# qiutang98/chord

Hardware: AMD Instinct MI355X
Metric: Gtri/s into 4K 64-bit visbuffer (higher is better)
Workload: dtype f32+u64; 1 GPU; street_4k_hzb; scene_triangles_lod0=2799616, objects=352, hzb=True, cull=flat, parallelism=single

## Files before the change

### chord_amd/csrc/kernels_raster.hip

```cpp

#include "device_layer.h"
#include "device_math.h"

#include <algorithm>
#include <cstdlib>
#include <cstring>
#include <type_traits>

namespace chord {

#define GUARD_BAND 1024.0f
#define LDS_VERTS 256
#define TILE CHORD_TILE
#define TILE_SHIFT CHORD_TILE_SHIFT
#define TPITCH (TILE + 1)
#define SMALL_AREA 256
#define TC_STRIDE CHORD_TILECOUNT_STRIDE
#define TC_BLOCKS 1u
#define TC_TICKET 2u
#ifndef CHORD_MASKED_FUSED
#define CHORD_MASKED_FUSED 1
#endif
#define TC_MASKED 3u

struct RasterParams {
    const uint32_t* count; const ChordDrawCmd* cmds;
    uint32_t cmdCap;
    uint32_t* leftCount; ChordDrawCmd* leftCmds;
    const DObjFrame* objFrame; const DObjStatic* objStatic;
    const DMeshlet* meshlets; const uint32_t* meshletData; const float* positions;
    const DMaterial* materials; const uint8_t* texAlpha; const float* texcoords;
    unsigned long long* vis;
    float* depthOut;
    float W, H; int32_t Wi, Hi;
    ShardInfo shard;
    TriRec* tris; uint32_t triCap;
    TriRecC* trisC; uint32_t triCapC;
    uint32_t* tileCount; uint32_t* tileBins; uint32_t binCap; uint32_t tilesX, tilesY;
    uint32_t* binPool; uint32_t binPoolChunks; uint32_t* binPoolCount;
    unsigned long long* binChunkTab; uint32_t binStamp; uint32_t binMaxChunks;
    unsigned long long* blockPool; uint32_t blockCap;
    uint32_t blockForce;
    ClipTri* clipTris; uint32_t clipTriCap; uint32_t pass;
    uint32_t* largeList; uint32_t largeCap;
    DeviceCounters* counters;
    uint2* tileOrder;
    unsigned long long* tileSlabs;
    uint32_t hzbFused;
    ChordHZBDesc hzbDesc;
    uint16_t* hzbMinA;
    uint16_t* hzbMinB; uint16_t* hzbMaxB;
    uint16_t* hzbExA;
    uint16_t* hzbExB;
    uint32_t* tileRange;
    unsigned long long* tileClocks;
    unsigned long long* tilePhase;
    uint32_t depthOnly, depthClamp;
    float biasConst, biasSlope;
    uint32_t clearTiles;
    uint32_t* binHint;
    uint32_t* countHint;
    uint32_t slotHot;
    uint32_t* hotTiles;
    uint32_t tileSlots;
    uint32_t tileSplitMin, tileSliceLen;
    uint2* tileOrderNext;
    uint32_t orderAll;
    uint32_t orderKept;
    uint32_t* heavyHint;
    uint32_t* tileTouched;
    uint32_t debug;
};
#define ABL(p, flag) (RASTER_ABLATION && ((p).debug & (flag)) != 0u)
#define DBG_NO_PIXELS   1u
#define DBG_NO_BIN      2u
#define DBG_TILE_CLOCKS 16u
#define DBG_NO_OUT      128u
#define DBG_NO_HZB      256u
#define DBG_SETUP_CLOCKS 512u
#define DBG_NO_VIS_STORE 1024u
#define DBG_NO_SPLIT    2048u
#define DBG_NO_TINY     32u
#define DBG_TILE_EXIT   64u
#define DBG_NO_ENTRY    8192u
#define DBG_NO_BATCH    16384u
#define DBG_NO_UNITS    4096u
#define DBG_SKIP_LIGHT  1048576u
#define DBG_SKIP_HEAVY  2097152u

template <typename T>
__device__ __forceinline__ T scalar_load(const T* ptr)
{
    return *reinterpret_cast<const __attribute__((address_space(4))) T*>(reinterpret_cast<uintptr_t>(ptr));
}
__device__ __forceinline__ const RasterParams* kernel_args()
{
    unsigned long long kp = (unsigned long long)__builtin_amdgcn_kernarg_segment_ptr();
    asm volatile("" : "+s"(kp));
    return reinterpret_cast<const RasterParams*>(kp);
}

__device__ __forceinline__ uint32_t mbcnt64(unsigned long long m) { return __builtin_amdgcn_mbcnt_hi((uint32_t)(m >> 32), __builtin_amdgcn_mbcnt_lo((uint32_t)m, 0u)); }
__device__ __forceinline__ int32_t bcast(int32_t v, int src) { return __builtin_amdgcn_readlane(v, src); }
__device__ __forceinline__ uint32_t bcast(uint32_t v, int src) { return (uint32_t)__builtin_amdgcn_readlane((int)v, src); }
__device__ __forceinline__ float bcast(float v, int src) { return __int_as_float(__builtin_amdgcn_readlane(__float_as_int(v), src)); }

__device__ __forceinline__ bool owns_tile(const ShardInfo& s, int32_t tx, int32_t ty)
{
    if (s.ranks <= 1) return true;
    return shard_owns_tile(s, (uint32_t)tx, (uint32_t)ty);
}
__device__ __forceinline__ bool owns_rect(const ShardInfo& s, int32_t px0, int32_t py0, int32_t px1, int32_t py1)
{
    if (s.ranks <= 1) return true;
    return shard_owns_any_tile(s, (uint32_t)px0 >> TILE_SHIFT, (uint32_t)py0 >> TILE_SHIFT, (uint32_t)px1 >> TILE_SHIFT, (uint32_t)py1 >> TILE_SHIFT);
}

__device__ __forceinline__ bool in_fast_volume_xy(const f4& h)
{
    return h.w > 0.0f && (GUARD_BAND * h.w + h.x) >= 0.0f && (GUARD_BAND * h.w - h.x) >= 0.0f &&
           (GUARD_BAND * h.w + h.y) >= 0.0f && (GUARD_BAND * h.w - h.y) >= 0.0f;
}

__device__ __forceinline__ bool in_fast_volume(const f4& h)
{
    return h.w > 0.0f && (h.w - h.z) >= 0.0f && h.z >= 0.0f &&
           (GUARD_BAND * h.w + h.x) >= 0.0f && (GUARD_BAND * h.w - h.x) >= 0.0f &&
           (GUARD_BAND * h.w + h.y) >= 0.0f && (GUARD_BAND * h.w - h.y) >= 0.0f;
}

struct TriSetup {
    int32_t X[3], Y[3];
    float d0, e1, e2, invA;
    int32_t px0, py0, px1, py1;
    int64_t area;
    int32_t s;
    uint32_t payload;
};

__device__ __forceinline__ bool narrow_extent(const TriSetup& ts)
{
    const int32_t extX = max(ts.X[0], max(ts.X[1], ts.X[2])) - min(ts.X[0], min(ts.X[1], ts.X[2]));
    const int32_t extY = max(ts.Y[0], max(ts.Y[1], ts.Y[2])) - min(ts.Y[0], min(ts.Y[1], ts.Y[2]));
    return extX <= (1 << 14) && extY <= (1 << 14);
}

__device__ __forceinline__ bool fits_compact(const TriSetup& ts)
{
    return narrow_extent(ts);
}

__device__ __forceinline__ void write_record_c(TriRecC* dst, const TriSetup& ts, const float d[3])
{
    TriRecC r;
    r.X0 = ts.X[0]; r.Y0 = ts.Y[0];
    r.dX1 = (int16_t)(ts.X[1] - ts.X[0]); r.dY1 = (int16_t)(ts.Y[1] - ts.Y[0]);
    r.dX2 = (int16_t)(ts.X[2] - ts.X[0]); r.dY2 = (int16_t)(ts.Y[2] - ts.Y[0]);
    r.d[0] = d[0]; r.d[1] = d[1]; r.d[2] = d[2];
    r.payload = ts.payload;
    *dst = r;
}

__device__ __forceinline__ bool tri_setup(TriSetup& ts, bool twoSided, int32_t Wi, int32_t Hi)
{
    const int32_t dx1 = ts.X[1] - ts.X[0], dy1 = ts.Y[1] - ts.Y[0], dx2 = ts.X[2] - ts.X[0], dy2 = ts.Y[2] - ts.Y[0];
    int64_t area2;
    const bool small = (uint32_t)(dx1 + 32767) < 65535u && (uint32_t)(dy1 + 32767) < 65535u &&
                       (uint32_t)(dx2 + 32767) < 65535u && (uint32_t)(dy2 + 32767) < 65535u;
    const bool allSmall = __ballot(!small) == 0ull;
    if (allSmall) area2 = (int64_t)(__mul24(dx1, dy2) - __mul24(dx2, dy1));
    else area2 = (int64_t)dx1 * (int64_t)dy2 - (int64_t)dx2 * (int64_t)dy1;
    if (area2 == 0) return false;
    if (!twoSided && area2 > 0) return false;
    ts.s = area2 < 0 ? -1 : 1;
    ts.area = area2 < 0 ? -area2 : area2;
    const int32_t minX = min(ts.X[0], min(ts.X[1], ts.X[2])), maxX = max(ts.X[0], max(ts.X[1], ts.X[2]));
    const int32_t minY = min(ts.Y[0], min(ts.Y[1], ts.Y[2])), maxY = max(ts.Y[0], max(ts.Y[1], ts.Y[2]));
    ts.px0 = max(0, (minX + 127) >> 8);
    ts.py0 = max(0, (minY + 127) >> 8);
    ts.px1 = min(Wi - 1, (maxX - 128) >> 8);
    ts.py1 = min(Hi - 1, (maxY - 128) >> 8);
    if (ts.px1 < ts.px0 || ts.py1 < ts.py0) return false;
    if (allSmall) ts.invA = 1.0f / (float)(int32_t)ts.area;
    else ts.invA = 1.0f / (float)(double)ts.area;
    return true;
}

__device__ __forceinline__ float depth_bias(const TriSetup& ts, const float d[3], float biasConst, float biasSlope)
{
    const int64_t s = ts.s;
    const float invA = ts.invA;
    const int64_t a1 = -s * (int64_t)(ts.Y[0] - ts.Y[2]), b1 = s * (int64_t)(ts.X[0] - ts.X[2]);
    const int64_t a2 = -s * (int64_t)(ts.Y[1] - ts.Y[0]), b2 = s * (int64_t)(ts.X[1] - ts.X[0]);
    const float e1 = d[1] - d[0], e2 = d[2] - d[0];
    const float dzdx = ((float)(double)(a1 * 256) * invA) * e1 + ((float)(double)(a2 * 256) * invA) * e2;
    const float dzdy = ((float)(double)(b1 * 256) * invA) * e1 + ((float)(double)(b2 * 256) * invA) * e2;
    const float m = fmaxf(fabsf(dzdx), fabsf(dzdy));
    const float mz = fmaxf(fabsf(d[0]), fmaxf(fabsf(d[1]), fabsf(d[2])));
    const int32_t e = (int32_t)((__float_as_uint(mz) >> 23) & 0xFFu) - 23;
    const float r = (e > 0 && e < 255) ? __uint_as_float((uint32_t)e << 23) : 0.0f;
    return biasSlope * m + biasConst * r;
}

__device__ __forceinline__ void tri_setup_from_compact(TriSetup& ts, const TriRecC& r, int32_t Wi, int32_t Hi)
{
    ts.X[0] = r.X0; ts.Y[0] = r.Y0;
    ts.X[1] = r.X0 + r.dX1; ts.Y[1] = r.Y0 + r.dY1;
    ts.X[2] = r.X0 + r.dX2; ts.Y[2] = r.Y0 + r.dY2;
    ts.payload = r.payload;
    const int32_t area2 = (int32_t)r.dX1 * (int32_t)r.dY2 - (int32_t)r.dX2 * (int32_t)r.dY1;
    ts.s = area2 < 0 ? -1 : 1;
    ts.invA = 1.0f / (float)(area2 < 0 ? -area2 : area2);
    ts.d0 = r.d[0]; ts.e1 = r.d[1] - r.d[0]; ts.e2 = r.d[2] - r.d[0];
    const int32_t minX = min(ts.X[0], min(ts.X[1], ts.X[2])), maxX = max(ts.X[0], max(ts.X[1], ts.X[2]));
    const int32_t minY = min(ts.Y[0], min(ts.Y[1], ts.Y[2])), maxY = max(ts.Y[0], max(ts.Y[1], ts.Y[2]));
    ts.px0 = max(0, (minX + 127) >> 8);
    ts.py0 = max(0, (minY + 127) >> 8);
    ts.px1 = min(Wi - 1, (maxX - 128) >> 8);
    ts.py1 = min(Hi - 1, (maxY - 128) >> 8);
    ts.area = 0;
}

__device__ __forceinline__ void tri_setup_from_record(TriSetup& ts, const TriRec& r, int32_t Wi, int32_t Hi)
{
#pragma unroll
    for (int i = 0; i < 3; i++) { ts.X[i] = r.X[i]; ts.Y[i] = r.Y[i]; }
    ts.payload = r.payload;
    ts.s = (r.twoSided & 2u) ? -1 : 1;
    ts.invA = __uint_as_float(r.pad);
    ts.d0 = r.d[0]; ts.e1 = r.d[1] - r.d[0]; ts.e2 = r.d[2] - r.d[0];
    const int32_t minX = min(ts.X[0], min(ts.X[1], ts.X[2])), maxX = max(ts.X[0], max(ts.X[1], ts.X[2]));
    const int32_t minY = min(ts.Y[0], min(ts.Y[1], ts.Y[2])), maxY = max(ts.Y[0], max(ts.Y[1], ts.Y[2]));
    ts.px0 = max(0, (minX + 127) >> 8);
    ts.py0 = max(0, (minY + 127) >> 8);
    ts.px1 = min(Wi - 1, (maxX - 128) >> 8);
    ts.py1 = min(Hi - 1, (maxY - 128) >> 8);
    ts.area = 0;
}



struct RecordEmitParams {
    DeviceCounters* counters; ClipTri* clipTris; uint32_t clipTriCap; uint32_t pass;
    TriRec* tris; uint32_t triCap; TriRecC* trisC; uint32_t triCapC; uint32_t* largeList; uint32_t largeCap;
    uint32_t* tileCount; uint32_t* tileBins; uint32_t binCap; uint32_t tilesX;
    uint32_t* binPool; uint32_t binPoolChunks; uint32_t* binPoolCount;
    unsigned long long* binChunkTab; uint32_t binStamp; uint32_t binMaxChunks;
    uint32_t* tileTouched;
    ShardInfo shard;
};
__device__ __forceinline__ RecordEmitParams load_record_emit_params()
{
    const RasterParams* q = kernel_args();
    RecordEmitParams e;
    e.counters = scalar_load(&q->counters); e.clipTris = scalar_load(&q->clipTris); e.clipTriCap = scalar_load(&q->clipTriCap); e.pass = scalar_load(&q->pass);
    e.tris = scalar_load(&q->tris); e.triCap = scalar_load(&q->triCap); e.trisC = scalar_load(&q->trisC); e.triCapC = scalar_load(&q->triCapC);
    e.largeList = scalar_load(&q->largeList); e.largeCap = scalar_load(&q->largeCap);
    e.tileCount = scalar_load(&q->tileCount); e.tileBins = scalar_load(&q->tileBins); e.binCap = scalar_load(&q->binCap); e.tilesX = scalar_load(&q->tilesX);
    e.binPool = scalar_load(&q->binPool); e.binPoolChunks = scalar_load(&q->binPoolChunks); e.binPoolCount = scalar_load(&q->binPoolCount);
    e.binChunkTab = scalar_load(&q->binChunkTab); e.binStamp = scalar_load(&q->binStamp); e.binMaxChunks = scalar_load(&q->binMaxChunks);
    e.tileTouched = scalar_load(&q->tileTouched);
    e.shard.ranks = scalar_load(&q->shard.ranks); e.shard.rank = scalar_load(&q->shard.rank); e.shard.slotsPerRank = 0u; e.shard.tilesX = 0u;
    e.shard.ownedRows = scalar_load(&q->shard.ownedRows); e.shard.tileSlot = nullptr;
    return e;
}

struct BinElect { int leader; uint32_t rank, group; };

__device__ __forceinline__ BinElect wave_bin_elect(bool has, uint32_t tile, uint32_t lane)
{
    BinElect e; e.leader = 0; e.rank = 0; e.group = 0;
    unsigned long long todo = __ballot(has);
    const unsigned long long lt = (1ull << lane) - 1ull;
    while (todo) {
        const int l = __ffsll((long long)todo) - 1;
        const uint32_t k = bcast(tile, l);
        const unsigned long long same = __ballot(has && tile == k);
        if (has && tile == k) { e.leader = l; e.rank = (uint32_t)__popcll(same & lt); e.group = (uint32_t)__popcll(same); }
        todo &= ~same;
    }
    return e;
}

__device__ __forceinline__ uint32_t bin_capacity(const RasterParams& p) { return p.binCap + p.binMaxChunks * CHORD_BIN_CHUNK; }

template <class P>
__device__ __forceinline__ void bin_alloc(const P& p, uint32_t tile, uint32_t slot)
{
    if (slot == 0u && p.tileTouched) atomicOr(&p.tileTouched[tile >> 5], 1u << (tile & 31u));
#ifdef EXP_NO_CHUNKS
    return;
#endif
    if (slot < p.binCap) return;
    const uint32_t o = slot - p.binCap, j = o >> CHORD_BIN_CHUNK_SHIFT;
    if (j >= p.binMaxChunks || (o & (CHORD_BIN_CHUNK - 1u)) != 0u) return;
    uint32_t id = atomicAdd(p.binPoolCount, 1u);
    if (id >= p.binPoolChunks) { id = CHORD_BIN_CHUNK_INVALID; atomicOr(&p.counters->overflow, 1u); }
    __hip_atomic_store(p.binChunkTab + (__umul24(tile, p.binMaxChunks) + j), ((unsigned long long)p.binStamp << 32) | id,
                       __ATOMIC_RELAXED, __HIP_MEMORY_SCOPE_AGENT);
}

template <class P>
__device__ __forceinline__ void bin_put(const P& p, uint32_t tile, uint32_t slot, uint32_t gi)
{
#ifdef EXP_NO_CHUNKS
    slot &= p.binCap - 1u;
#endif
    if (slot < p.binCap) { p.tileBins[__umul24(tile, p.binCap) + slot] = gi; return; }
    const uint32_t o = slot - p.binCap, j = o >> CHORD_BIN_CHUNK_SHIFT;
    if (j >= p.binMaxChunks) { atomicOr(&p.counters->overflow, 1u); return; }
    const unsigned long long* ent = p.binChunkTab + (__umul24(tile, p.binMaxChunks) + j);
    const unsigned long long stamp = (unsigned long long)p.binStamp << 32;
    unsigned long long e = 0;
    uint32_t spins = 0;
    for (;;) {
        e = __hip_atomic_load(ent, __ATOMIC_RELAXED, __HIP_MEMORY_SCOPE_AGENT);
        if ((e & 0xFFFFFFFF00000000ull) == stamp) break;
        if (++spins > (1u << 20)) { atomicOr(&p.counters->overflow, 4u); return; }
        __builtin_amdgcn_s_sleep(4);
    }
    const uint32_t id = (uint32_t)e;
    if (id != CHORD_BIN_CHUNK_INVALID) p.binPool[((size_t)id << CHORD_BIN_CHUNK_SHIFT) + (o & (CHORD_BIN_CHUNK - 1u))] = gi;
}

__device__ __forceinline__ void bin_store(const RasterParams& p, uint32_t tile, uint32_t slot, uint32_t gi)
{
    bin_alloc(p, tile, slot);
    bin_put(p, tile, slot, gi);
}

struct BinTicket {
    uint32_t tileA[4], tileB[4], slotA[4], slotB[4];
    uint32_t has;
    uint32_t eA[4], eB[4];
};

template <class P>
__device__ __forceinline__ void wave_bin_issue(const P& p, bool emitA, const TriSetup& tsA, bool emitB, const TriSetup& tsB,
                                               uint32_t lane, BinTicket& k, const bool masked = false)
{
    auto tile_of = [&](const TriSetup& ts, int r, bool emit, uint32_t& tile) -> bool {
        const int32_t tx0 = ts.px0 >> TILE_SHIFT, tx1 = ts.px1 >> TILE_SHIFT, ty0 = ts.py0 >> TILE_SHIFT, ty1 = ts.py1 >> TILE_SHIFT;
        const int32_t tx = (r & 1) ? tx1 : tx0, ty = (r & 2) ? ty1 : ty0;
        bool has = emit && !((r & 1) && tx1 == tx0) && !((r & 2) && ty1 == ty0);
        if (has) has = owns_tile(p.shard, tx, ty);
        tile = has ? __umul24((uint32_t)ty, p.tilesX) + (uint32_t)tx : 0u;
        return has;
    };
    k.has = 0u;
#pragma unroll
    for (int r = 0; r < 4; r++) {
        k.slotA[r] = 0u; k.slotB[r] = 0u;
        if (tile_of(tsA, r, emitA, k.tileA[r])) k.has |= 1u << r;
        if (tile_of(tsB, r, emitB, k.tileB[r])) k.has |= 16u << r;
    }
#pragma unroll
    for (int r = 0; r < 4; r++) {
        const BinElect a = wave_bin_elect((k.has & (1u << r)) != 0u, k.tileA[r], lane);
        const BinElect b = wave_bin_elect((k.has & (16u << r)) != 0u, k.tileB[r], lane);
        k.eA[r] = (uint32_t)a.leader | a.rank << 8; k.eB[r] = (uint32_t)b.leader | b.rank << 8;
        if ((k.has & (1u << r)) && (int)lane == a.leader) k.slotA[r] = atomicAdd(&p.tileCount[(size_t)k.tileA[r] * TC_STRIDE], a.group);
        if ((k.has & (16u << r)) && (int)lane == b.leader) k.slotB[r] = atomicAdd(&p.tileCount[(size_t)k.tileB[r] * TC_STRIDE], b.group);
    }
    if (masked) {
#pragma unroll
        for (int r = 0; r < 4; r++) {
            if ((k.has & (1u << r)) && lane == (k.eA[r] & 0xFFu)) p.tileCount[(size_t)k.tileA[r] * TC_STRIDE + TC_MASKED] = 1u;
            if ((k.has & (16u << r)) && lane == (k.eB[r] & 0xFFu)) p.tileCount[(size_t)k.tileB[r] * TC_STRIDE + TC_MASKED] = 1u;
        }
    }
}

template <class P>
__device__ __forceinline__ void wave_bin_commit(const P& p, BinTicket& k, bool okA, uint32_t giA, bool okB, uint32_t giB)
{
#pragma unroll
    for (int r = 0; r < 4; r++) {
        k.slotA[r] = __shfl(k.slotA[r], (int)(k.eA[r] & 0xFFu), 64) + (k.eA[r] >> 8);
        k.slotB[r] = __shfl(k.slotB[r], (int)(k.eB[r] & 0xFFu), 64) + (k.eB[r] >> 8);
    }
    if (k.has) {
#pragma unroll
        for (int r = 0; r < 4; r++) {
            if (k.has & (1u << r)) bin_alloc(p, k.tileA[r], k.slotA[r]);
            if (k.has & (16u << r)) bin_alloc(p, k.tileB[r], k.slotB[r]);
        }
    }
#pragma unroll
    for (int r = 0; r < 4; r++) {
        if (okA && (k.has & (1u << r))) bin_put(p, k.tileA[r], k.slotA[r], giA);
        if (okB && (k.has & (16u << r))) bin_put(p, k.tileB[r], k.slotB[r], giB);
    }
}

__device__ __forceinline__ bool touches_many_tiles(const TriSetup& ts)
{
    return ((ts.px1 >> TILE_SHIFT) - (ts.px0 >> TILE_SHIFT)) > 1 || ((ts.py1 >> TILE_SHIFT) - (ts.py0 >> TILE_SHIFT)) > 1;
}

__device__ __forceinline__ void write_record(TriRec* dst, const TriSetup& ts, const float d[3], bool twoSided, bool masked = false)
{
    TriRec r;
#pragma unroll
    for (int i = 0; i < 3; i++) { r.X[i] = ts.X[i]; r.Y[i] = ts.Y[i]; r.d[i] = d[i]; }
    r.payload = ts.payload;
    r.twoSided = (twoSided ? 1u : 0u) | (ts.s < 0 ? 2u : 0u) | (masked ? 4u : 0u);
    r.pad = __float_as_uint(ts.invA);
    *dst = r;
}

__device__ __forceinline__ bool filter_is_linear(uint32_t f)
{
    return f == CHORD_FILTER_LINEAR || f == CHORD_FILTER_LINEAR_MIPMAP_NEAREST || f == CHORD_FILTER_LINEAR_MIPMAP_LINEAR;
}

__device__ __forceinline__ uint32_t mask_level_filter(const DMaterial& m, int64_t absArea2, const float u[3], const float v[3])
{
    uint32_t level = 0u;
    bool linear = filter_is_linear(m.magFilter);
    if (m.texOffset != 0xFFFFFFFFu) {
        const float texels = (float)m.texWidth * (float)m.texHeight;
        const float auv = fabsf((u[1] - u[0]) * (v[2] - v[0]) - (u[2] - u[0]) * (v[1] - v[0])) * texels;
        const float apx = (float)(double)absArea2 * (1.0f / 65536.0f);
        const float ratio = auv / apx;
        if (ratio >= 1.0f) {
            const int32_t e = (int32_t)((__float_as_uint(ratio) >> 23) & 0xFFu) - 127;
            level = min((uint32_t)(e >> 1), m.texMips - 1u);
            linear = filter_is_linear(m.minFilter);
        }
    }
    return level | (linear ? 256u : 0u);
}

__device__ __forceinline__ void write_mask_ext(TriRec* slot, const DMaterial* mp, uint32_t material, int64_t absArea2,
                                               const float u[3], const float v[3], const float w[3])
{
    DMaterial m;
    m.texOffset = mp->texOffset; m.texWidth = mp->texWidth; m.texHeight = mp->texHeight; m.texMips = mp->texMips;
    m.minFilter = mp->minFilter; m.magFilter = mp->magFilter; m.wrapS = mp->wrapS; m.wrapT = mp->wrapT;
    m.alphaFactor = mp->alphaFactor; m.alphaCutOff = mp->alphaCutOff;
    TriRecMaskExt e;
#pragma unroll
    for (int i = 0; i < 3; i++) { e.iw[i] = 1.0f / w[i]; e.uw[i] = u[i] * e.iw[i]; e.vw[i] = v[i] * e.iw[i]; }
    e.levelFilter = mask_level_filter(m, absArea2, u, v);
    (void)material;
    const uint32_t level = e.levelFilter & 0xFFu;
    e.levelBase = 0xFFFFFFFFu; e.dims = 0u; e.magicS = e.biasS = e.magicT = e.biasT = 0u;
    if (m.texOffset != 0xFFFFFFFFu) {
        const DMatLevel L = mp->levels[level];
        e.levelBase = L.base; e.dims = L.dims;
        e.magicS = L.magicS; e.biasS = L.biasS; e.magicT = L.magicT; e.biasT = L.biasT;
    }
    e.wraps = (m.wrapS & 0xFFFFu) | m.wrapT << 16;
    e.alphaFactor = m.alphaFactor; e.alphaCutOff = m.alphaCutOff;
    uint4* dst = reinterpret_cast<uint4*>(slot);
    const uint4* src = reinterpret_cast<const uint4*>(&e);
    dst[0] = src[0]; dst[1] = src[1]; dst[2] = src[2]; dst[3] = src[3];
    reinterpret_cast<uint32_t*>(slot)[16] = e.biasS; reinterpret_cast<uint32_t*>(slot)[17] = e.magicT; reinterpret_cast<uint32_t*>(slot)[18] = e.biasT;
}

#ifndef EXP_MASKED
#define EXP_MASKED 0
#endif
__device__ __forceinline__ int32_t period_mod(int32_t i, int32_t period, uint32_t magic, uint32_t bias)
{
    if ((EXP_MASKED & 4) || magic == 0u) return i & (period - 1);
    const uint32_t iu = (uint32_t)i + bias;
    uint32_t r = iu - __umulhi(iu, magic) * (uint32_t)period;
    if (r >= (uint32_t)period) r -= (uint32_t)period;
    return (int32_t)r;
}
__device__ __forceinline__ int32_t wrap_index(int32_t i, int32_t n, uint32_t mode, uint32_t magic, uint32_t bias)
{
    if (mode == CHORD_WRAP_CLAMP_TO_EDGE) return i < 0 ? 0 : (i > n - 1 ? n - 1 : i);
    if (mode == CHORD_WRAP_MIRRORED_REPEAT) {
        const int32_t m = period_mod(i, 2 * n, magic, bias);
        return m < n ? m : 2 * n - 1 - m;
    }
    return period_mod(i, n, magic, bias);
}

__device__ __forceinline__ void wrap_pair(int32_t i, int32_t n, uint32_t mode, uint32_t magic, uint32_t bias, int32_t& w0, int32_t& w1)
{
    if (mode == CHORD_WRAP_CLAMP_TO_EDGE) {
        w0 = i < 0 ? 0 : (i > n - 1 ? n - 1 : i);
        w1 = i + 1 < 0 ? 0 : (i + 1 > n - 1 ? n - 1 : i + 1);
        return;
    }
    const bool mirror = mode == CHORD_WRAP_MIRRORED_REPEAT;
    const int32_t period = mirror ? 2 * n : n;
    const int32_t m = period_mod(i, period, magic, bias);
    const int32_t m1 = m + 1 == period ? 0 : m + 1;
    w0 = mirror ? (m < n ? m : 2 * n - 1 - m) : m;
    w1 = mirror ? (m1 < n ? m1 : 2 * n - 1 - m1) : m1;
}

__device__ __forceinline__ int32_t texel_floor(float x)
{
    if (!(fabsf(x) < 1.0e9f)) return 0;
    return (int32_t)floorf(x);
}

struct AlphaLevel {
    const uint8_t* base;
    int32_t W, H;
    float fW, fH;
    uint32_t wrapS, wrapT;
    uint32_t magicS, biasS, magicT, biasT;
    bool linear;
};
__device__ __forceinline__ AlphaLevel alpha_level(const uint8_t* __restrict__ texAlpha, const TriRecMaskExt& e)
{
    const uint32_t levelBase = e.levelBase, dims = e.dims;
    AlphaLevel a;
    a.base = nullptr; a.W = 1; a.H = 1; a.fW = 1.0f; a.fH = 1.0f; a.wrapS = e.wraps & 0xFFFFu; a.wrapT = e.wraps >> 16; a.linear = (e.levelFilter & 256u) != 0u;
    a.magicS = e.magicS; a.biasS = e.biasS; a.magicT = e.magicT; a.biasT = e.biasT;
    if (levelBase == 0xFFFFFFFFu) return a;
    a.W = (int32_t)(dims & 0xFFFFu) + 1; a.H = (int32_t)(dims >> 16) + 1;
    a.fW = (float)a.W; a.fH = (float)a.H;
    a.base = texAlpha + levelBase;
    return a;
}
__device__ __forceinline__ float sample_alpha(const AlphaLevel& t, float u, float v)
{
    if (!t.base) return 1.0f;
    if (EXP_MASKED & 1) return 1.0f;
    if (!t.linear || (EXP_MASKED & 2)) {
        const int32_t ix = wrap_index(texel_floor(u * t.fW), t.W, t.wrapS, t.magicS, t.biasS), iy = wrap_index(texel_floor(v * t.fH), t.H, t.wrapT, t.magicT, t.biasT);
        return (float)t.base[iy * t.W + ix] * (1.0f / 255.0f);
    }
    const float x = u * t.fW - 0.5f, y = v * t.fH - 0.5f;
    const int32_t x0 = texel_floor(x), y0 = texel_floor(y);
    float fx = x - (float)x0, fy = y - (float)y0;
    if (!(fabsf(x) < 1.0e9f)) fx = 0.0f;
    if (!(fabsf(y) < 1.0e9f)) fy = 0.0f;
    int32_t ix0, ix1, iy0, iy1;
    wrap_pair(x0, t.W, t.wrapS, t.magicS, t.biasS, ix0, ix1);
    wrap_pair(y0, t.H, t.wrapT, t.magicT, t.biasT, iy0, iy1);
    const float a00 = (float)t.base[iy0 * t.W + ix0] * (1.0f / 255.0f), a10 = (float)t.base[iy0 * t.W + ix1] * (1.0f / 255.0f);
    const float a01 = (float)t.base[iy1 * t.W + ix0] * (1.0f / 255.0f), a11 = (float)t.base[iy1 * t.W + ix1] * (1.0f / 255.0f);
    const float top = a00 + (a10 - a00) * fx, bot = a01 + (a11 - a01) * fx;
    return top + (bot - top) * fy;
}

__device__ __forceinline__ void setup_emit_mask_ext(const RasterParams& p, TriRec* slot, uint32_t triWord, const float uv[6],
                                                 const float* lW, uint32_t material, int64_t absArea2)
{
    float u[3], v[3], w[3];
#pragma unroll
    for (int i = 0; i < 3; i++) {
        u[i] = uv[2 * i]; v[i] = uv[2 * i + 1];
        w[i] = lW[(triWord >> (8 * i)) & 0xFFu];
    }
    write_mask_ext(slot, &p.materials[material], material, absArea2, u, v, w);
}

template <int PITCH>
__device__ __forceinline__ void tile_raster_narrow(unsigned long long* tile, const TriSetup& ts, int32_t ox, int32_t oy,
                                                   int32_t x0, int32_t y0, int32_t x1, int32_t y1, bool noPixels, const bool clampZ);

__device__ __forceinline__ void wave_min2_max2(int32_t& a, int32_t& b, int32_t& c, int32_t& d)
{
#define DPP_STEP(ctrl)                                                \
    "v_min_i32_dpp %0, %0, %0 " ctrl "\n\t"                           \
    "v_min_i32_dpp %1, %1, %1 " ctrl "\n\t"                           \
    "v_max_i32_dpp %2, %2, %2 " ctrl "\n\t"                           \
    "v_max_i32_dpp %3, %3, %3 " ctrl "\n\t"
    asm volatile("s_nop 1\n\t"
                 DPP_STEP("quad_perm:[1,0,3,2] row_mask:0xf bank_mask:0xf")
                 DPP_STEP("quad_perm:[2,3,0,1] row_mask:0xf bank_mask:0xf")
                 DPP_STEP("row_ror:4 row_mask:0xf bank_mask:0xf")
                 DPP_STEP("row_ror:8 row_mask:0xf bank_mask:0xf")
                 DPP_STEP("row_bcast:15 row_mask:0xa bank_mask:0xf")
                 DPP_STEP("row_bcast:31 row_mask:0xc bank_mask:0xf")
                 "s_nop 0"
                 : "+v"(a), "+v"(b), "+v"(c), "+v"(d));
#undef DPP_STEP
    a = __builtin_amdgcn_readlane(a, 63); b = __builtin_amdgcn_readlane(b, 63);
    c = __builtin_amdgcn_readlane(c, 63); d = __builtin_amdgcn_readlane(d, 63);
}

__device__ __forceinline__ void wave_sum2(uint32_t& a, uint32_t& b)
{
#define DPP_STEP(ctrl)                                                \
    "v_add_u32_dpp %0, %0, %0 " ctrl "\n\t"                           \
    "v_add_u32_dpp %1, %1, %1 " ctrl "\n\t"
    asm volatile("s_nop 1\n\t"
                 DPP_STEP("quad_perm:[1,0,3,2] row_mask:0xf bank_mask:0xf") "s_nop 0\n\t"
                 DPP_STEP("quad_perm:[2,3,0,1] row_mask:0xf bank_mask:0xf") "s_nop 0\n\t"
                 DPP_STEP("row_ror:4 row_mask:0xf bank_mask:0xf") "s_nop 0\n\t"
                 DPP_STEP("row_ror:8 row_mask:0xf bank_mask:0xf") "s_nop 0\n\t"
                 DPP_STEP("row_bcast:15 row_mask:0xa bank_mask:0xf") "s_nop 0\n\t"
                 DPP_STEP("row_bcast:31 row_mask:0xc bank_mask:0xf")
                 "s_nop 0"
                 : "+v"(a), "+v"(b));
#undef DPP_STEP
    a = (uint32_t)__builtin_amdgcn_readlane((int)a, 63); b = (uint32_t)__builtin_amdgcn_readlane((int)b, 63);
}

enum { K_NONE = 0, K_EMIT = 1, K_CLIP = 2 };
#define WIN CHORD_BLOCK_WIN
#define DBG_NO_BLOCKS 32768u
#define DBG_FORCE_BLOCKS 65536u
#define DBG_FORCE_HOT 262144u

template <bool MASKED>
__device__ __forceinline__ void raster_setup_body(const RasterParams& p, const ChordDrawCmd* __restrict__ cmds, const uint32_t count, float (*sVert)[4][LDS_VERTS],
                                                  const uint32_t firstCmd0, const uint32_t firstCmd1, const uint32_t firstCmd2, const bool firstCmdValid)
{
    const uint32_t lane = threadIdx.x & 63u, wave = threadIdx.x >> 6;
    float* lX = sVert[0][wave]; float* lY = sVert[1][wave]; float* lW = sVert[2][wave];
    float* lU = sVert[3][wave]; float* lV = sVert[4][wave]; float* lD = sVert[5][wave];

    const uint32_t listShard = (blockIdx.x * 4u + wave) % CHORD_LIST_SHARDS;

    struct Header {
        uint32_t objectId, meshletId, slot, V, T, dataOffset, vertexBase, matFlags;
        bool twoSided;
    };
    auto header_of = [&](uint32_t objectId, uint32_t meshletId, uint32_t slot) -> Header {
        Header h;
        h.objectId = objectId; h.meshletId = meshletId; h.slot = slot;
        const RasterParams* q = kernel_args();
        const DMeshlet* __restrict__ mm = &scalar_load(&q->meshlets)[h.meshletId];
        const uint32_t vt = scalar_load(&mm->vertexTriangleCount);
        h.V = vt & 0xFFu; h.T = (vt >> 8) & 0xFFu;
        h.dataOffset = scalar_load(&mm->dataOffset);
        h.vertexBase = scalar_load(&mm->vertexBase);
        h.matFlags = scalar_load(&scalar_load(&q->objStatic)[h.objectId].matFlags);
        h.twoSided = (h.matFlags & CHORD_MATFLAG_TWO_SIDED) != 0u;
        if (CHORD_MATFLAG_ALPHA(h.matFlags) >= CHORD_ALPHA_BLEND) h.T = 0u;
        return h;
    };
    auto load_header = [&](uint32_t i) -> Header {
        const uint32_t k = __builtin_amdgcn_readfirstlane(min(i, count - 1u));
        const uint32_t* __restrict__ cw = reinterpret_cast<const uint32_t*>(cmds + k);
        return header_of(scalar_load(cw), scalar_load(cw + 1), scalar_load(cw + 2));
    };
    auto mvp_of = [&](uint32_t objectId) -> Mat4 {
        Mat4 m;
        const float* __restrict__ mv = scalar_load(&kernel_args()->objFrame)[objectId].mvp;
#pragma unroll
        for (int r = 0; r < 4; r++)
#pragma unroll
            for (int cc = 0; cc < 4; cc++) m.r[r][cc] = scalar_load(mv + r * 4 + cc);
        return m;
    };
    const uint32_t stride = gridDim.x * 4u;
    uint32_t c = blockIdx.x * 4u + wave;
    if (c >= count) return;
    Header hdr = firstCmdValid ? header_of(firstCmd0, firstCmd1, firstCmd2) : load_header(c);
    Header hdrN = load_header(c + stride);
    Mat4 mvpNext = mvp_of(hdr.objectId);
    uint32_t t0 = 0, t1 = 0;
    float pax, pay, paz, pbx, pby, pbz;
    {
        const uint32_t* __restrict__ md = scalar_load(&kernel_args()->meshletData);
        const float* __restrict__ ps = scalar_load(&kernel_args()->positions);
        const uint32_t ia = md[hdr.dataOffset + min(lane, max(hdr.V, 1u) - 1u)] + hdr.vertexBase;
        const uint32_t ib = md[hdr.dataOffset + min(lane + 64u, max(hdr.V, 1u) - 1u)] + hdr.vertexBase;
        if (lane < hdr.T) t0 = md[hdr.dataOffset + hdr.V + lane];
        if (lane + 64u < hdr.T) t1 = md[hdr.dataOffset + hdr.V + 64u + lane];
        const float* __restrict__ pa = ps + (size_t)(ia * 3u);
        const float* __restrict__ pb = ps + (size_t)(ib * 3u);
        pax = pa[0]; pay = pa[1]; paz = pa[2]; pbx = pb[0]; pby = pb[1]; pbz = pb[2];
    }
    const bool sprof = RASTER_PROFILE && (p.debug & DBG_SETUP_CLOCKS) != 0;
    unsigned long long sph[5] = {0, 0, 0, 0, 0}, stp = sprof ? wall_clock64() : 0ull;
#define SPHASE(i) do { if (sprof) { const unsigned long long tn = wall_clock64(); sph[i] += tn - stp; stp = tn; } } while (0)
    const uint32_t laneTop = lane;
    for (; c < count; c += stride) {
        uint32_t lane = laneTop;
        asm volatile("" : "+v"(lane));
        const uint32_t slot = hdr.slot, V = hdr.V, T = hdr.T, dataOffset = hdr.dataOffset, vertexBase = hdr.vertexBase;
        const bool twoSided = hdr.twoSided || p.depthOnly != 0u;
        const bool masked = MASKED && CHORD_MATFLAG_ALPHA(hdr.matFlags) == CHORD_ALPHA_MASK;
        const Mat4 mvp = mvpNext;
        const uint32_t triWord[2] = {t0, t1};

        if (sprof) { volatile uint32_t sink = V + T; (void)sink; }
        SPHASE(0);
        bool notFast = false;
        auto vertex = [&](uint32_t i, float x, float y, float z) {
            const f4 h = mul_mv(mvp, x, y, z, 1.0f);
            const float aw = fabsf(h.w);
            lX[i] = h.x; lY[i] = h.y; lW[i] = h.w;
            lU[i] = h.x / aw * 0.5f + 0.5f;
            lV[i] = h.y / aw * -0.5f + 0.5f;
            const bool fast = p.depthClamp ? in_fast_volume_xy(h) : in_fast_volume(h);
            lD[i] = fast ? h.z / h.w : __builtin_nanf("");
            notFast = notFast || !fast;
        };
        if (lane < V) vertex(lane, pax, pay, paz);
        if (lane + 64u < V) vertex(lane + 64u, pbx, pby, pbz);
        for (uint32_t i = lane + 128u; i < V; i += 64u) {
            const float* __restrict__ pp = scalar_load(&kernel_args()->positions) + (size_t)(scalar_load(&kernel_args()->meshletData)[dataOffset + i] + vertexBase) * 3;
            vertex(i, pp[0], pp[1], pp[2]);
        }
        const bool allFast = __ballot(notFast) == 0ull;
        __builtin_amdgcn_fence(__ATOMIC_RELEASE, "wavefront");
        __builtin_amdgcn_wave_barrier();
        __builtin_amdgcn_fence(__ATOMIC_ACQUIRE, "wavefront");
        SPHASE(1);
        const uint32_t* __restrict__ mdN = scalar_load(&kernel_args()->meshletData);
        const uint32_t nia = mdN[hdrN.dataOffset + min(lane, max(hdrN.V, 1u) - 1u)] + hdrN.vertexBase;
        const uint32_t nib = mdN[hdrN.dataOffset + min(lane + 64u, max(hdrN.V, 1u) - 1u)] + hdrN.vertexBase;
        const uint32_t nt0 = lane < hdrN.T ? mdN[hdrN.dataOffset + hdrN.V + lane] : 0u;
        const uint32_t nt1 = lane + 64u < hdrN.T ? mdN[hdrN.dataOffset + hdrN.V + 64u + lane] : 0u;

        float uvA[6] = {0.0f, 0.0f, 0.0f, 0.0f, 0.0f, 0.0f}, uvB[6] = {0.0f, 0.0f, 0.0f, 0.0f, 0.0f, 0.0f};
        if (MASKED && masked && scalar_load(&kernel_args()->texcoords) != nullptr) {
            const float* __restrict__ tc = scalar_load(&kernel_args()->texcoords);
            const uint32_t* __restrict__ mdT = scalar_load(&kernel_args()->meshletData);
#pragma unroll
            for (int i = 0; i < 3; i++) {
                if (lane < T) { const size_t vi = (size_t)(mdT[dataOffset + ((t0 >> (8 * i)) & 0xFFu)] + vertexBase) * 2; uvA[2 * i] = tc[vi]; uvA[2 * i + 1] = tc[vi + 1]; }
                if (lane + 64u < T) { const size_t vi = (size_t)(mdT[dataOffset + ((t1 >> (8 * i)) & 0xFFu)] + vertexBase) * 2; uvB[2 * i] = tc[vi]; uvB[2 * i + 1] = tc[vi + 1]; }
            }
        }
        int kindA = K_NONE, kindB = K_NONE;
        TriSetup tsA, tsB;
        float dA[3] = {0.0f, 0.0f, 0.0f}, dB[3] = {0.0f, 0.0f, 0.0f};
        tsA.px0 = tsA.py0 = tsA.px1 = tsA.py1 = 0; tsB.px0 = tsB.py0 = tsB.px1 = tsB.py1 = 0;
#pragma unroll
        for (int half = 0; half < 2; half++) {
            const uint32_t t = (uint32_t)half * 64u + lane;
            int kind = K_NONE;
            TriSetup ts;
            ts.px0 = ts.py0 = ts.px1 = ts.py1 = 0;
            float d[3] = {0.0f, 0.0f, 0.0f};
            if (t < T) {
                const uint32_t packedIdx = triWord[half];
                const uint32_t i0 = packedIdx & 0xFFu, i1 = (packedIdx >> 8) & 0xFFu, i2 = (packedIdx >> 16) & 0xFFu;
                const float x0 = lX[i0], y0 = lY[i0], w0 = lW[i0];
                const float x1 = lX[i1], y1 = lY[i1], w1 = lW[i1];
                const float x2 = lX[i2], y2 = lY[i2], w2 = lW[i2];
                bool culled = false;
                if (!twoSided) {
                    const float det = (x0 * (y1 * w2 - w1 * y2) - y0 * (x1 * w2 - w1 * x2)) + w0 * (x1 * y2 - y1 * x2);
                    culled = det <= 0.0f;
                }
                culled = culled || (w0 <= 0.0f && w1 <= 0.0f && w2 <= 0.0f);
                const float u0 = lU[i0], v0 = lV[i0], u1 = lU[i1], v1 = lV[i1], u2 = lU[i2], v2 = lV[i2];
                const float maxU = fmaxf(u0, fmaxf(u1, u2)), maxV = fmaxf(v0, fmaxf(v1, v2));
                const float minU = fminf(u0, fminf(u1, u2)), minV = fminf(v0, fminf(v1, v2));
                culled = culled || ((minU >= 1.0f || minV >= 1.0f) || (maxU <= 0.0f || maxV <= 0.0f));
                culled = culled || (rintf(minU * p.W) == rintf(maxU * p.W) || rintf(minV * p.H) == rintf(maxV * p.H));
                if (!culled) {
                    d[0] = lD[i0]; d[1] = lD[i1]; d[2] = lD[i2];
                    ts.payload = p.depthOnly ? 0u : encode_triangle_instance(t, slot);
                    if (!allFast && (d[0] != d[0] || d[1] != d[1] || d[2] != d[2])) {
                        kind = K_CLIP;
                    } else {
                        ts.X[0] = (int32_t)rintf((u0 * p.W) * 256.0f); ts.Y[0] = (int32_t)rintf((v0 * p.H) * 256.0f);
                        ts.X[1] = (int32_t)rintf((u1 * p.W) * 256.0f); ts.Y[1] = (int32_t)rintf((v1 * p.H) * 256.0f);
                        ts.X[2] = (int32_t)rintf((u2 * p.W) * 256.0f); ts.Y[2] = (int32_t)rintf((v2 * p.H) * 256.0f);
                        if (tri_setup(ts, twoSided, p.Wi, p.Hi) && owns_rect(p.shard, ts.px0, ts.py0, ts.px1, ts.py1)) {
                            kind = K_EMIT;
                            if (p.biasConst != 0.0f || p.biasSlope != 0.0f) { const float o = depth_bias(ts, d, p.biasConst, p.biasSlope); d[0] += o; d[1] += o; d[2] += o; }
                        }
                    }
                }
            }
            if (ABL(p, DBG_NO_BIN)) kind = K_NONE;
            if (half == 0) { kindA = kind; tsA = ts; dA[0] = d[0]; dA[1] = d[1]; dA[2] = d[2]; }
            else           { kindB = kind; tsB = ts; dB[0] = d[0]; dB[1] = d[1]; dB[2] = d[2]; }
        }
        SPHASE(2);
        const float* __restrict__ psN = scalar_load(&kernel_args()->positions);
        const float* __restrict__ npa = psN + (size_t)(nia * 3u);
        const float* __restrict__ npb = psN + (size_t)(nib * 3u);
        const float nax = npa[0], nay = npa[1], naz = npa[2], nbx = npb[0], nby = npb[1], nbz = npb[2];
        {
            const unsigned long long lt = (1ull << lane) - 1ull;
            const unsigned long long cmA = __ballot(kindA == K_CLIP), cmB = __ballot(kindB == K_CLIP);
            const unsigned long long emA = __ballot(kindA == K_EMIT), emB = __ballot(kindB == K_EMIT);
            const bool cpA = kindA == K_EMIT && !masked && fits_compact(tsA), cpB = kindB == K_EMIT && !masked && fits_compact(tsB);
            const uint32_t wSlots = masked ? 1u + CHORD_MASK_EXT_SLOTS : 1u;
            const unsigned long long ecA = __ballot(cpA), ecB = __ballot(cpB);
            const unsigned long long ewA = emA & ~ecA, ewB = emB & ~ecB;
            const bool lgA = kindA == K_EMIT && touches_many_tiles(tsA), lgB = kindB == K_EMIT && touches_many_tiles(tsB);
            const unsigned long long lmA = __ballot(lgA), lmB = __ballot(lgB);
            const uint32_t nClip = (uint32_t)(__popcll(cmA) + __popcll(cmB));
            const uint32_t nEc = (uint32_t)(__popcll(ecA) + __popcll(ecB)), nEw = (uint32_t)(__popcll(ewA) + __popcll(ewB));
            const uint32_t nLg = (uint32_t)(__popcll(lmA) + __popcll(lmB));
            {
            const RecordEmitParams e = load_record_emit_params();
            uint32_t cbase = 0, ebaseC = 0, ebaseW = 0, lbase = 0;
            if (lane == 0) {
                if (nClip) cbase = atomicAdd(&e.counters->clipTriCount[p.pass], nClip);
                if (nEc) ebaseC = atomicAdd(&e.counters->triCountC[listShard * CHORD_SHARD_STRIDE], nEc);
                if (nEw) ebaseW = atomicAdd(&e.counters->triCount[listShard * CHORD_SHARD_STRIDE], nEw * wSlots);
                if (nLg) lbase = atomicAdd(&e.counters->largeCount[p.pass][listShard * CHORD_SHARD_STRIDE], nLg);
            }
            BinTicket ticket;
            if (emA | emB) wave_bin_issue(e, kindA == K_EMIT && !lgA, tsA, kindB == K_EMIT && !lgB, tsB, lane, ticket, MASKED && masked);
            cbase = bcast(cbase, 0); ebaseC = bcast(ebaseC, 0); ebaseW = bcast(ebaseW, 0); lbase = bcast(lbase, 0);
            SPHASE(3);
            mvpNext = mvp_of(hdrN.objectId);
            if (kindA == K_CLIP) {
                const uint32_t k = cbase + (uint32_t)__popcll(cmA & lt);
                if (k < e.clipTriCap) { ClipTri ct; ct.objectId = hdr.objectId; ct.meshletId = hdr.meshletId; ct.slot = hdr.slot; ct.tri = lane; e.clipTris[k] = ct; }
                else atomicOr(&e.counters->overflow, 2u);
            }
            if (kindB == K_CLIP) {
                const uint32_t k = cbase + (uint32_t)__popcll(cmA) + (uint32_t)__popcll(cmB & lt);
                if (k < e.clipTriCap) { ClipTri ct; ct.objectId = hdr.objectId; ct.meshletId = hdr.meshletId; ct.slot = hdr.slot; ct.tri = lane + 64u; e.clipTris[k] = ct; }
                else atomicOr(&e.counters->overflow, 2u);
            }
            uint32_t giA = 0, giB = 0;
            bool okA = false, okB = false;
            if (cpA) {
                const uint32_t li = ebaseC + (uint32_t)__popcll(ecA & lt);
                if (li < e.triCapC) { giA = listShard * e.triCapC + li; write_record_c(&e.trisC[giA], tsA, dA); okA = true; }
                else atomicOr(&e.counters->overflow, 1u);
            } else if (kindA == K_EMIT) {
                const uint32_t li = ebaseW + wSlots * (uint32_t)__popcll(ewA & lt);
                if (li + wSlots <= e.triCap) {
                    giA = listShard * e.triCap + li; write_record(&e.tris[giA], tsA, dA, twoSided, masked);
                    if (MASKED && masked) setup_emit_mask_ext(p, &e.tris[giA + 1u], triWord[0], uvA, lW, CHORD_MATFLAG_MATERIAL(hdr.matFlags), tsA.area);
                    giA |= (MASKED && masked) ? CHORD_REC_MASKED : CHORD_REC_WIDE; okA = true;
                } else atomicOr(&e.counters->overflow, 1u);
            }
            if (cpB) {
                const uint32_t li = ebaseC + (uint32_t)__popcll(ecA) + (uint32_t)__popcll(ecB & lt);
                if (li < e.triCapC) { giB = listShard * e.triCapC + li; write_record_c(&e.trisC[giB], tsB, dB); okB = true; }
                else atomicOr(&e.counters->overflow, 1u);
            } else if (kindB == K_EMIT) {
                const uint32_t li = ebaseW + wSlots * ((uint32_t)__popcll(ewA) + (uint32_t)__popcll(ewB & lt));
                if (li + wSlots <= e.triCap) {
                    giB = listShard * e.triCap + li; write_record(&e.tris[giB], tsB, dB, twoSided, masked);
                    if (MASKED && masked) setup_emit_mask_ext(p, &e.tris[giB + 1u], triWord[1], uvB, lW, CHORD_MATFLAG_MATERIAL(hdr.matFlags), tsB.area);
                    giB |= (MASKED && masked) ? CHORD_REC_MASKED : CHORD_REC_WIDE; okB = true;
                } else atomicOr(&e.counters->overflow, 1u);
            }
            if (emA | emB) wave_bin_commit(e, ticket, okA, giA, okB, giB);
            if (lgA && okA) {
                const uint32_t k = lbase + (uint32_t)__popcll(lmA & lt);
                if (k < e.largeCap) e.largeList[(size_t)listShard * e.largeCap + k] = giA & CHORD_REC_WIDE_INDEX; else atomicOr(&e.counters->overflow, 1u);
            }
            if (lgB && okB) {
                const uint32_t k = lbase + (uint32_t)__popcll(lmA) + (uint32_t)__popcll(lmB & lt);
                if (k < e.largeCap) e.largeList[(size_t)listShard * e.largeCap + k] = giB & CHORD_REC_WIDE_INDEX; else atomicOr(&e.counters->overflow, 1u);
            }
            }
        }
        __builtin_amdgcn_fence(__ATOMIC_RELEASE, "wavefront");
        __builtin_amdgcn_wave_barrier();
        hdr = hdrN;
        hdrN = load_header(c + 2u * stride);
        t0 = nt0; t1 = nt1;
        pax = nax; pay = nay; paz = naz; pbx = nbx; pby = nby; pbz = nbz;
        SPHASE(4);
    }
    if (sprof && lane == 0u) {
        const uint32_t w = blockIdx.x * 4u + wave;
        if (w < CHORD_MAX_TILES * 8u / 5u) for (int i = 0; i < 5; i++) p.tilePhase[(size_t)w * 5u + i] = sph[i];
    }
#undef SPHASE
}

struct SetupHeader { uint32_t objectId, meshletId, slot, V, T, dataOffset, vertexBase, matFlags; };

struct BlockEmitParams {
    uint32_t* tileCount; uint32_t* tileBins; uint32_t binCap;
    uint32_t* binPool; uint32_t binPoolChunks; uint32_t* binPoolCount;
    unsigned long long* binChunkTab; uint32_t binStamp; uint32_t binMaxChunks;
    unsigned long long* blockPool; uint32_t blockCap;
    DeviceCounters* counters;
    uint32_t* tileTouched;
};
__device__ __forceinline__ BlockEmitParams load_block_emit_params()
{
    const RasterParams* q = kernel_args();
    BlockEmitParams e;
    e.tileCount = scalar_load(&q->tileCount); e.tileBins = scalar_load(&q->tileBins); e.binCap = scalar_load(&q->binCap);
    e.binPool = scalar_load(&q->binPool); e.binPoolChunks = scalar_load(&q->binPoolChunks); e.binPoolCount = scalar_load(&q->binPoolCount);
    e.binChunkTab = scalar_load(&q->binChunkTab); e.binStamp = scalar_load(&q->binStamp); e.binMaxChunks = scalar_load(&q->binMaxChunks);
    e.blockPool = scalar_load(&q->blockPool); e.blockCap = scalar_load(&q->blockCap);
    e.counters = scalar_load(&q->counters);
    e.tileTouched = scalar_load(&q->tileTouched);
    return e;
}

#define WAVE_LDS_SYNC() do { __builtin_amdgcn_fence(__ATOMIC_RELEASE, "wavefront"); __builtin_amdgcn_wave_barrier(); __builtin_amdgcn_fence(__ATOMIC_ACQUIRE, "wavefront"); } while (0)

__device__ __forceinline__ int classify_triangle(const RasterParams& p, uint32_t t, uint32_t T, uint32_t packedIdx, bool twoSided, bool allFast,
                                                 const float* lX, const float* lY, const float* lW, const float* lU, const float* lV, const float* lD,
                                                 const int32_t* lSX, const int32_t* lSY, uint32_t& boxX, uint32_t& boxY, bool& narrow)
{
    boxX = 0u; boxY = 0u; narrow = false;
    if (t >= T) return K_NONE;
    const uint32_t i0 = packedIdx & 0xFFu, i1 = (packedIdx >> 8) & 0xFFu, i2 = (packedIdx >> 16) & 0xFFu;
    const float w0 = lW[i0], w1 = lW[i1], w2 = lW[i2];
    bool culled = false;
    if (!twoSided) {
        const float x0 = lX[i0], y0 = lY[i0], x1 = lX[i1], y1 = lY[i1], x2 = lX[i2], y2 = lY[i2];
        const float det = (x0 * (y1 * w2 - w1 * y2) - y0 * (x1 * w2 - w1 * x2)) + w0 * (x1 * y2 - y1 * x2);
        culled = det <= 0.0f;
    }
    culled = culled || (w0 <= 0.0f && w1 <= 0.0f && w2 <= 0.0f);
    const float u0 = lU[i0], v0 = lV[i0], u1 = lU[i1], v1 = lV[i1], u2 = lU[i2], v2 = lV[i2];
    const float maxU = fmaxf(u0, fmaxf(u1, u2)), maxV = fmaxf(v0, fmaxf(v1, v2));
    const float minU = fminf(u0, fminf(u1, u2)), minV = fminf(v0, fminf(v1, v2));
    culled = culled || ((minU >= 1.0f || minV >= 1.0f) || (maxU <= 0.0f || maxV <= 0.0f));
    culled = culled || (rintf(minU * p.W) == rintf(maxU * p.W) || rintf(minV * p.H) == rintf(maxV * p.H));
    if (culled) return K_NONE;
    if (!allFast) { const float d0 = lD[i0], d1 = lD[i1], d2 = lD[i2]; if (d0 != d0 || d1 != d1 || d2 != d2) return K_CLIP; }
    const int32_t X0 = lSX[i0], Y0 = lSY[i0], X1 = lSX[i1], Y1 = lSY[i1], X2 = lSX[i2], Y2 = lSY[i2];
    const int32_t minX = min(X0, min(X1, X2)), maxX = max(X0, max(X1, X2));
    const int32_t minY = min(Y0, min(Y1, Y2)), maxY = max(Y0, max(Y1, Y2));
    if (maxX - minX > (1 << 14) || maxY - minY > (1 << 14)) return K_EMIT;
    narrow = true;
    const int32_t area2 = __mul24(X1 - X0, Y2 - Y0) - __mul24(X2 - X0, Y1 - Y0);
    if (area2 == 0 || (!twoSided && area2 > 0)) return K_NONE;
    const int32_t px0 = max(0, (minX + 127) >> 8), py0 = max(0, (minY + 127) >> 8);
    const int32_t px1 = min(p.Wi - 1, (maxX - 128) >> 8), py1 = min(p.Hi - 1, (maxY - 128) >> 8);
    if (px1 < px0 || py1 < py0) return K_NONE;
    boxX = (uint32_t)px0 | ((uint32_t)px1 << 16); boxY = (uint32_t)py0 | ((uint32_t)py1 << 16);
    return K_EMIT;
}

__device__ __forceinline__ void resolve_entry(const RasterParams& p, uint32_t entry, uint32_t boxX, uint32_t boxY, uint32_t slot,
                                              const int32_t* lSX, const int32_t* lSY, const float* lD, unsigned long long* win,
                                              int32_t bx0, int32_t by0)
{
    const uint32_t i0 = entry & 0xFFu, i1 = (entry >> 8) & 0xFFu, i2 = (entry >> 16) & 0xFFu, t = entry >> 24;
    TriSetup ts;
    ts.X[0] = lSX[i0]; ts.Y[0] = lSY[i0];
    ts.X[1] = lSX[i1]; ts.Y[1] = lSY[i1];
    ts.X[2] = lSX[i2]; ts.Y[2] = lSY[i2];
    const int32_t dx1 = ts.X[1] - ts.X[0], dy1 = ts.Y[1] - ts.Y[0], dx2 = ts.X[2] - ts.X[0], dy2 = ts.Y[2] - ts.Y[0];
    const int32_t area2 = __mul24(dx1, dy2) - __mul24(dx2, dy1);
    const int32_t area = area2 < 0 ? -area2 : area2;
    ts.s = area2 < 0 ? -1 : 1;
    ts.area = (int64_t)area;
    ts.invA = 1.0f / (float)area;
    ts.px0 = (int32_t)(boxX & 0xFFFFu); ts.px1 = (int32_t)(boxX >> 16);
    ts.py0 = (int32_t)(boxY & 0xFFFFu); ts.py1 = (int32_t)(boxY >> 16);
    float d[3] = {lD[i0], lD[i1], lD[i2]};
    if (p.biasConst != 0.0f || p.biasSlope != 0.0f) { const float o = depth_bias(ts, d, p.biasConst, p.biasSlope); d[0] += o; d[1] += o; d[2] += o; }
    ts.payload = p.depthOnly ? 0u : encode_triangle_instance(t, slot);
    ts.d0 = d[0]; ts.e1 = d[1] - d[0]; ts.e2 = d[2] - d[0];
    if (p.depthClamp != 0u) tile_raster_narrow<WIN>(win, ts, bx0, by0, ts.px0, ts.py0, ts.px1, ts.py1, false, true);
    else tile_raster_narrow<WIN>(win, ts, bx0, by0, ts.px0, ts.py0, ts.px1, ts.py1, false, false);
}

#define SLOT_CACHE 32u
#define SLOT_HOT 65536u
#ifndef SLOT_AHEAD
#define SLOT_AHEAD 8u
#endif
#ifndef SLOT_AHEAD_VERY_HOT
#define SLOT_AHEAD_VERY_HOT 32u
#endif
#define SLOT_VERY_HOT 262144u
struct SlotCache { uint32_t key[SLOT_CACHE], next[SLOT_CACHE], end[SLOT_CACHE]; uint32_t pend; };

#ifndef BLOCKS_LDS_VERTS
#define BLOCKS_LDS_VERTS 128
#endif
template <bool HOT>
__device__ __forceinline__ void raster_setup_blocks_body(const RasterParams& p, const uint32_t count, float (*sVert)[4][BLOCKS_LDS_VERTS], int32_t (*sSnap)[4][BLOCKS_LDS_VERTS],
                                                         unsigned long long (*sWin)[WIN * WIN], SlotCache* slotCaches)
{
    const uint32_t lane = threadIdx.x & 63u, wave = threadIdx.x >> 6;
    SlotCache& sc = slotCaches[HOT ? wave : 0u];
    if (HOT && lane < SLOT_CACHE) { sc.key[lane] = 0u; sc.next[lane] = 0u; sc.end[lane] = 0u; }
    if (HOT) {
        const uint32_t* __restrict__ hl = scalar_load(&kernel_args()->hotTiles);
        WAVE_LDS_SYNC();
        if (hl) {
            const uint32_t nHot = min(hl[0], (uint32_t)CHORD_HOT_TILES);
            if (lane < nHot) {
                const uint32_t e = hl[1u + lane], tile = e & 0xFFFu, ci = tile & (SLOT_CACHE - 1u);
                const uint32_t pos = (e >> 31) ? SLOT_VERY_HOT : 0u;
                sc.key[ci] = tile + 1u; sc.next[ci] = pos; sc.end[ci] = pos;
            }
        }
        WAVE_LDS_SYNC();
    }
    float* lX = sVert[0][wave]; float* lY = sVert[1][wave]; float* lW = sVert[2][wave];
    float* lU = sVert[3][wave]; float* lV = sVert[4][wave]; float* lD = sVert[5][wave];
    int32_t* lSX = sSnap[0][wave]; int32_t* lSY = sSnap[1][wave];
    unsigned long long* win = sWin[wave];
    const uint32_t listShard = (blockIdx.x * 4u + wave) % CHORD_LIST_SHARDS;

    auto kq = [&]() -> const RasterParams* { return kernel_args(); };
    auto header_at = [&](uint32_t i) -> SetupHeader {
        const uint32_t k = __builtin_amdgcn_readfirstlane(min(i, count - 1u));
        SetupHeader h;
        const RasterParams* q = kq();
        const uint32_t* __restrict__ cw = reinterpret_cast<const uint32_t*>(scalar_load(&q->cmds) + k);
        h.objectId = scalar_load(cw); h.meshletId = scalar_load(cw + 1); h.slot = scalar_load(cw + 2);
        const DMeshlet* __restrict__ mm = &scalar_load(&q->meshlets)[h.meshletId];
        const uint32_t vt = scalar_load(&mm->vertexTriangleCount);
        h.V = vt & 0xFFu; h.T = (vt >> 8) & 0xFFu;
        h.dataOffset = scalar_load(&mm->dataOffset);
        h.vertexBase = scalar_load(&mm->vertexBase);
        h.matFlags = scalar_load(&scalar_load(&q->objStatic)[h.objectId].matFlags);
        if (CHORD_MATFLAG_ALPHA(h.matFlags) >= CHORD_ALPHA_BLEND) h.T = 0u;
        return h;
    };
    auto mvp_of = [&](uint32_t objectId) -> Mat4 {
        Mat4 m;
        const float* __restrict__ mv = scalar_load(&kq()->objFrame)[objectId].mvp;
#pragma unroll
        for (int r = 0; r < 4; r++)
#pragma unroll
            for (int cc = 0; cc < 4; cc++) m.r[r][cc] = scalar_load(mv + r * 4 + cc);
        return m;
    };
    const uint32_t stride = gridDim.x * 4u;
    uint32_t c = blockIdx.x * 4u + wave;
    if (c >= count) return;
    SetupHeader hdr = header_at(c);
    SetupHeader hdrN = header_at(c + stride);
    uint32_t t0 = 0, t1 = 0;
    float pax, pay, paz, pbx, pby, pbz;
    {
        const uint32_t* __restrict__ md = scalar_load(&kq()->meshletData);
        const float* __restrict__ ps = scalar_load(&kq()->positions);
        const uint32_t ia = md[hdr.dataOffset + min(lane, max(hdr.V, 1u) - 1u)] + hdr.vertexBase;
        const uint32_t ib = md[hdr.dataOffset + min(lane + 64u, max(hdr.V, 1u) - 1u)] + hdr.vertexBase;
        if (lane < hdr.T) t0 = md[hdr.dataOffset + hdr.V + lane];
        if (lane + 64u < hdr.T) t1 = md[hdr.dataOffset + hdr.V + 64u + lane];
        const float* __restrict__ pa = ps + (size_t)(ia * 3u);
        const float* __restrict__ pb = ps + (size_t)(ib * 3u);
        pax = pa[0]; pay = pa[1]; paz = pa[2]; pbx = pb[0]; pby = pb[1]; pbz = pb[2];
    }
    const bool sprof = RASTER_PROFILE && (p.debug & DBG_SETUP_CLOCKS) != 0;
    unsigned long long sph[5] = {0, 0, 0, 0, 0}, stp = sprof ? wall_clock64() : 0ull;
#define SPHASE(i) do { if (sprof) { const unsigned long long tn = wall_clock64(); sph[i] += tn - stp; stp = tn; } } while (0)
    for (; c < count; c += stride) {
        const uint32_t V = hdr.V, T = hdr.T, dataOffset = hdr.dataOffset, vertexBase = hdr.vertexBase;
        const bool twoSided = (hdr.matFlags & CHORD_MATFLAG_TWO_SIDED) != 0u || p.depthOnly != 0u;
        const bool masked = CHORD_MATFLAG_ALPHA(hdr.matFlags) == CHORD_ALPHA_MASK;
        if (sprof) { volatile uint32_t sink = V + T; (void)sink; }
        SPHASE(0);
        const bool tooBig = V > (uint32_t)BLOCKS_LDS_VERTS;
        (void)dataOffset; (void)vertexBase;
        bool notFast = false;
        if (!tooBig) {
            const Mat4 mvp = mvp_of(hdr.objectId);
            auto vertex = [&](uint32_t i, float x, float y, float z) {
                const f4 h = mul_mv(mvp, x, y, z, 1.0f);
                const float aw = fabsf(h.w);
                lX[i] = h.x; lY[i] = h.y; lW[i] = h.w;
                const float u = h.x / aw * 0.5f + 0.5f, v = h.y / aw * -0.5f + 0.5f;
                lU[i] = u; lV[i] = v;
                lSX[i] = (int32_t)rintf((u * p.W) * 256.0f); lSY[i] = (int32_t)rintf((v * p.H) * 256.0f);
                const bool fast = p.depthClamp ? in_fast_volume_xy(h) : in_fast_volume(h);
                lD[i] = fast ? h.z / h.w : __builtin_nanf("");
                notFast = notFast || !fast;
            };
            if (lane < V) vertex(lane, pax, pay, paz);
            if (lane + 64u < V) vertex(lane + 64u, pbx, pby, pbz);
#if BLOCKS_LDS_VERTS > 128
            for (uint32_t i = lane + 128u; i < V; i += 64u) {
                const float* __restrict__ pp = scalar_load(&kq()->positions) + (size_t)(scalar_load(&kq()->meshletData)[dataOffset + i] + vertexBase) * 3;
                vertex(i, pp[0], pp[1], pp[2]);
            }
#endif
        }
        const bool allFast = __ballot(notFast) == 0ull;
        WAVE_LDS_SYNC();
        SPHASE(1);
        const uint32_t* __restrict__ md = scalar_load(&kq()->meshletData);
        const uint32_t nia = md[hdrN.dataOffset + min(lane, max(hdrN.V, 1u) - 1u)] + hdrN.vertexBase;
        const uint32_t nib = md[hdrN.dataOffset + min(lane + 64u, max(hdrN.V, 1u) - 1u)] + hdrN.vertexBase;
        const uint32_t nt0 = lane < hdrN.T ? md[hdrN.dataOffset + hdrN.V + lane] : 0u;
        const uint32_t nt1 = lane + 64u < hdrN.T ? md[hdrN.dataOffset + hdrN.V + 64u + lane] : 0u;

        uint32_t bxA, byA, bxB, byB;
        bool nwA, nwB;
        int kindA = classify_triangle(p, lane, tooBig ? 0u : T, t0, twoSided, allFast, lX, lY, lW, lU, lV, lD, lSX, lSY, bxA, byA, nwA);
        int kindB = classify_triangle(p, lane + 64u, tooBig ? 0u : T, t1, twoSided, allFast, lX, lY, lW, lU, lV, lD, lSX, lSY, bxB, byB, nwB);
        if (ABL(p, DBG_NO_BIN)) { kindA = K_NONE; kindB = K_NONE; }
        SPHASE(2);
        const float* __restrict__ ps = scalar_load(&kq()->positions);
        const float* __restrict__ npa = ps + (size_t)(nia * 3u);
        const float* __restrict__ npb = ps + (size_t)(nib * 3u);
        const float nax = npa[0], nay = npa[1], naz = npa[2], nbx = npb[0], nby = npb[1], nbz = npb[2];

        const bool eA = kindA == K_EMIT, eB = kindB == K_EMIT;
        const unsigned long long emA = __ballot(eA), emB = __ballot(eB);
        const unsigned long long bad = __ballot(kindA == K_CLIP || kindB == K_CLIP || (eA && !nwA) || (eB && !nwB)) | (tooBig && T != 0u ? 1ull : 0ull);
        bool blocksDone = false;
        if (!masked && (emA | emB) != 0ull && bad == 0ull) {
            int32_t bx0 = min(eA ? (int32_t)(bxA & 0xFFFFu) : 0x7FFF, eB ? (int32_t)(bxB & 0xFFFFu) : 0x7FFF);
            int32_t by0 = min(eA ? (int32_t)(byA & 0xFFFFu) : 0x7FFF, eB ? (int32_t)(byB & 0xFFFFu) : 0x7FFF);
            int32_t bx1 = max(eA ? (int32_t)(bxA >> 16) : -1, eB ? (int32_t)(bxB >> 16) : -1);
            int32_t by1 = max(eA ? (int32_t)(byA >> 16) : -1, eB ? (int32_t)(byB >> 16) : -1);
            if (__ballot(bx1 - bx0 >= WIN || by1 - by0 >= WIN) == 0ull) {
                wave_min2_max2(bx0, by0, bx1, by1);
                const int32_t bw = bx1 - bx0 + 1, bh = by1 - by0 + 1;
                const uint32_t nE = (uint32_t)(__popcll(emA) + __popcll(emB));
                if (bw <= WIN && bh <= WIN && (uint32_t)(bw * bh + 8) * 8u <= nE * 36u) {
                    blocksDone = true;
                    const int32_t tx0 = bx0 >> TILE_SHIFT, tx1 = bx1 >> TILE_SHIFT, ty0 = by0 >> TILE_SHIFT, ty1 = by1 >> TILE_SHIFT;
                    const uint32_t r = lane & 3u;
                    const bool sx = (r & 1u) != 0u, sy = (r & 2u) != 0u;
                    const int32_t rx0 = sx ? tx1 << TILE_SHIFT : bx0, rx1 = (sx || tx1 == tx0) ? bx1 : (tx0 << TILE_SHIFT) + TILE - 1;
                    const int32_t ry0 = sy ? ty1 << TILE_SHIFT : by0, ry1 = (sy || ty1 == ty0) ? by1 : (ty0 << TILE_SHIFT) + TILE - 1;
                    const uint32_t rw = (uint32_t)(rx1 - rx0 + 1), rh = (uint32_t)(ry1 - ry0 + 1);
                    const bool has = lane < 4u && !(sx && tx1 == tx0) && !(sy && ty1 == ty0) && owns_tile(p.shard, sx ? tx1 : tx0, sy ? ty1 : ty0);
                    const uint32_t hasMask = (uint32_t)__ballot(has) & 15u;
                    const uint32_t gran = has ? (rw * rh + 2u) >> 1 : 0u;
                    const uint32_t g0 = bcast(gran, 0), g1 = bcast(gran, 1), g2 = bcast(gran, 2), g3 = bcast(gran, 3);
                    const uint32_t before = (r > 0u ? g0 : 0u) + (r > 1u ? g1 : 0u) + (r > 2u ? g2 : 0u), G = g0 + g1 + g2 + g3;
                    const uint32_t tile = __umul24((uint32_t)(sy ? ty1 : ty0), p.tilesX) + (uint32_t)(sx ? tx1 : tx0);
                    uint32_t gbase = 0, slot = 0;
                    const BlockEmitParams e = load_block_emit_params();
                    {
                        uint32_t ahead = 1u;
                        if (HOT) {
                            const uint32_t ci = tile & (SLOT_CACHE - 1u);
                            if (lane == 0u && has && sc.key[ci] == tile + 1u) {
                                const uint32_t nx = sc.next[ci];
                                if (nx < sc.end[ci]) { slot = nx; sc.next[ci] = nx + 1u; ahead = 0u; }
                                else ahead = nx >= SLOT_VERY_HOT ? SLOT_AHEAD_VERY_HOT : SLOT_AHEAD;
                            }
                            if (lane == 0u) sc.pend = ahead;
                        }
                        if (lane == 0u && G) gbase = atomicAdd(&e.counters->blockGranules[listShard * CHORD_SHARD_STRIDE], G);
                        if (has && ahead) slot = (uint32_t)atomicAdd(reinterpret_cast<unsigned long long*>(&e.tileCount[(size_t)tile * TC_STRIDE]), (unsigned long long)ahead * 0x100000001ull);
                    }
                    uint32_t* lList = reinterpret_cast<uint32_t*>(lX);
                    uint32_t* lBoxX = reinterpret_cast<uint32_t*>(lY);
                    uint32_t* lBoxY = reinterpret_cast<uint32_t*>(lW);
                    const uint32_t nA = (uint32_t)__popcll(emA);
                    WAVE_LDS_SYNC();
                    if (eA) { const uint32_t k = mbcnt64(emA); lList[k] = (t0 & 0xFFFFFFu) | lane << 24; lBoxX[k] = bxA; lBoxY[k] = byA; }
                    if (eB) { const uint32_t k = nA + mbcnt64(emB); lList[k] = (t1 & 0xFFFFFFu) | (lane + 64u) << 24; lBoxX[k] = bxB; lBoxY[k] = byB; }
#pragma unroll
                    for (int k = 0; k < WIN * WIN / 64; k++) win[lane + 64u * k] = 0ull;
                    WAVE_LDS_SYNC();
                    const bool anyPart = hasMask != 0u;
                    if (anyPart) {
                        if (lane < nE) resolve_entry(p, lList[lane], lBoxX[lane], lBoxY[lane], hdr.slot, lSX, lSY, lD, win, bx0, by0);
                        if (nE > 64u) {
                            __builtin_amdgcn_sched_barrier(0);
                            if (lane + 64u < nE) resolve_entry(p, lList[lane + 64u], lBoxX[lane + 64u], lBoxY[lane + 64u], hdr.slot, lSX, lSY, lD, win, bx0, by0);
                        }
                    }
                    WAVE_LDS_SYNC();
                    SPHASE(3);
                    gbase = bcast(gbase, 0);
                    const bool fits = gbase + G <= e.blockCap;
                    if (!fits && lane == 0u) atomicOr(&e.counters->overflow, 1u);
                    const uint32_t off = listShard * e.blockCap + gbase + before;
                    uint32_t drew = 1u;
                    if (HOT) {
                        if (lane == 0u) drew = sc.pend;
                        if (lane == 0u && has && drew) {
                            const uint32_t ci = tile & (SLOT_CACHE - 1u);
                            if (drew > 1u) {
                                sc.next[ci] = slot + 1u; sc.end[ci] = slot + drew;
                                for (uint32_t k = 1u; k < drew; k++) bin_alloc(e, tile, slot + k);
                            } else if (slot >= scalar_load(&kq()->slotHot) && (sc.key[ci] == 0u || sc.next[ci] >= sc.end[ci])) {
                                sc.key[ci] = tile + 1u; sc.next[ci] = 0u; sc.end[ci] = 0u;
                            }
                        }
                    }
                    if (has && drew) bin_alloc(e, tile, slot);
                    if (has && fits) bin_put(e, tile, slot, CHORD_REC_BLOCK | off);
                    if (fits) {
                        for (uint32_t q = 0; q < 4u; q++) {
                            if (!((hasMask >> q) & 1u)) continue;
                            const uint32_t qoff = bcast(off, (int)q), qw = bcast(rw, (int)q), qh = bcast(rh, (int)q);
                            const uint32_t qx = (uint32_t)bcast(rx0 - bx0, (int)q), qy = (uint32_t)bcast(ry0 - by0, (int)q);
                            const uint32_t qlx = (uint32_t)bcast(rx0 & (TILE - 1), (int)q), qly = (uint32_t)bcast(ry0 & (TILE - 1), (int)q);
                            const uint32_t n = qw * qh, gq = (n + 2u) >> 1;
                            const uint32_t rcp = (uint32_t)ceilf(65536.0f * __builtin_amdgcn_rcpf((float)qw));
                            const unsigned long long header = (unsigned long long)(qlx | qly << 6 | (qw - 1u) << 12 | (qh - 1u) << 16) | ((unsigned long long)rcp << 32);
                            ulonglong2* dst = reinterpret_cast<ulonglong2*>(e.blockPool + (size_t)qoff * 2u);
                            for (uint32_t g = lane; g < gq; g += 64u) {
                                const uint32_t j1 = 2u * g, j0 = g == 0u ? 0u : j1 - 1u;
                                const uint32_t row0 = __umul24(j0, rcp) >> 16, row1 = __umul24(j1, rcp) >> 16;
                                const unsigned long long w0 = g == 0u ? header : win[(qy + row0) * WIN + qx + (j0 - __umul24(row0, qw))];
                                const unsigned long long w1 = j1 < n ? win[(qy + row1) * WIN + qx + (j1 - __umul24(row1, qw))] : 0ull;
                                dst[g] = make_ulonglong2(w0, w1);
                            }
                        }
                    }
                }
            }
        }
        if (!blocksDone && ((emA | emB) != 0ull || bad != 0ull)) {
            if (lane == 0u) {
                const uint32_t k = atomicAdd(scalar_load(&kq()->leftCount), 1u);
                ChordDrawCmd cmd; cmd.objectId = hdr.objectId; cmd.meshletId = hdr.meshletId; cmd.slot = hdr.slot;
                scalar_load(&kq()->leftCmds)[k] = cmd;
            }
            SPHASE(3);
        }
        __builtin_amdgcn_fence(__ATOMIC_RELEASE, "wavefront");
        __builtin_amdgcn_wave_barrier();
        hdr = hdrN;
        hdrN = header_at(c + 2u * stride);
        t0 = nt0; t1 = nt1;
        pax = nax; pay = nay; paz = naz; pbx = nbx; pby = nby; pbz = nbz;
        SPHASE(4);
    }
    if (HOT) WAVE_LDS_SYNC();
    if (HOT && lane < SLOT_CACHE && sc.key[lane] != 0u && sc.next[lane] < sc.end[lane]) {
        const BlockEmitParams e = load_block_emit_params();
        for (uint32_t k = sc.next[lane]; k < sc.end[lane]; k++) bin_put(e, sc.key[lane] - 1u, k, 0xFFFFFFFFu);
    }
    if (sprof && lane == 0u) {
        const uint32_t w = blockIdx.x * 4u + wave;
        if (w < CHORD_MAX_TILES * 8u / 5u) for (int i = 0; i < 5; i++) p.tilePhase[(size_t)w * 5u + i] = sph[i];
    }
#undef SPHASE
}

__device__ __forceinline__ bool launch_is_dense(const RasterParams& p, uint32_t count)
{
    const unsigned long long pixels = (unsigned long long)p.Wi * (unsigned long long)p.Hi / (p.shard.ranks > 1u ? p.shard.ranks : 1u);
    return p.blockCap != 0u && p.leftCmds != nullptr && (p.blockForce != 0u || (unsigned long long)count * 16ull >= pixels);
}

#ifndef SETUP_MIN_WAVES
#define SETUP_MIN_WAVES 5
#endif
#ifndef BLOCKS_MIN_WAVES
#define BLOCKS_MIN_WAVES 6
#endif
#ifndef SETUP_MASKED_WAVES
#define SETUP_MASKED_WAVES 4
#endif
template <bool MASKED>
__global__ __launch_bounds__(256, MASKED ? SETUP_MASKED_WAVES : SETUP_MIN_WAVES) void raster_setup_kernel(RasterParams p)
{
    __shared__ float sVert[6][4][LDS_VERTS];
    const uint32_t c0 = __builtin_amdgcn_readfirstlane(min(blockIdx.x * 4u + (threadIdx.x >> 6), p.cmdCap - 1u));
    const uint32_t* __restrict__ cw = reinterpret_cast<const uint32_t*>(p.cmds + c0);
    const uint32_t f0 = scalar_load(cw), f1 = scalar_load(cw + 1), f2 = scalar_load(cw + 2);
    uint32_t count = *p.count;
    const ChordDrawCmd* cmds = p.cmds;
    bool firstValid = true;
    if (launch_is_dense(p, count)) { count = *p.leftCount; cmds = p.leftCmds; firstValid = false; }
    raster_setup_body<MASKED>(p, cmds, count, sVert, f0, f1, f2, firstValid);
}

template <bool HOT>
__global__ __launch_bounds__(256, BLOCKS_MIN_WAVES) void raster_setup_blocks_kernel(RasterParams p)
{
    __shared__ float sVert[6][4][BLOCKS_LDS_VERTS];
    __shared__ int32_t sSnap[2][4][BLOCKS_LDS_VERTS];
    __shared__ unsigned long long sWin[4][WIN * WIN];
    __shared__ SlotCache sSlots[HOT ? 4 : 1];
    const uint32_t count = *p.count;
    if (!launch_is_dense(p, count)) return;
    raster_setup_blocks_body<HOT>(p, count, sVert, sSnap, sWin, sSlots);
}

__device__ void bin_record_tiles(const RasterParams& p, const TriSetup& ts, uint32_t gi)
{
    const int ea[3] = {1, 2, 0}, eb[3] = {2, 0, 1};
    const int32_t tx0 = ts.px0 >> TILE_SHIFT, tx1 = ts.px1 >> TILE_SHIFT;
    const int32_t ty0 = ts.py0 >> TILE_SHIFT, ty1 = ts.py1 >> TILE_SHIFT;
    for (int32_t ty = ty0; ty <= ty1; ty++)
        for (int32_t tx = tx0; tx <= tx1; tx++) {
            const int32_t rx0 = max(ts.px0, tx << TILE_SHIFT), rx1 = min(ts.px1, (tx << TILE_SHIFT) + TILE - 1);
            const int32_t ry0 = max(ts.py0, ty << TILE_SHIFT), ry1 = min(ts.py1, (ty << TILE_SHIFT) + TILE - 1);
            bool hit = owns_tile(p.shard, tx, ty);
#pragma unroll
            for (int i = 0; i < 3; i++) {
                const int64_t dxe = (int64_t)(ts.X[eb[i]] - ts.X[ea[i]]), dye = (int64_t)(ts.Y[eb[i]] - ts.Y[ea[i]]);
                const int64_t a = -(int64_t)ts.s * dye, b = (int64_t)ts.s * dxe;
                const int64_t bias = (a > 0 || (a == 0 && b > 0)) ? 0 : -1;
                const int64_t cx = (int64_t)(a > 0 ? rx1 : rx0) * 256 + 128, cy = (int64_t)(b > 0 ? ry1 : ry0) * 256 + 128;
                hit = hit && !((int64_t)ts.s * (dxe * (cy - ts.Y[ea[i]]) - dye * (cx - ts.X[ea[i]])) + bias < 0);
            }
            if (!hit) continue;
            const uint32_t tile = (uint32_t)ty * p.tilesX + (uint32_t)tx;
            const uint32_t slot = atomicAdd(&p.tileCount[(size_t)tile * TC_STRIDE], 1u);
            bin_store(p, tile, slot, gi);
            if ((gi & 0xE0000000u) == CHORD_REC_MASKED) p.tileCount[(size_t)tile * TC_STRIDE + TC_MASKED] = 1u;
        }
}

__device__ __forceinline__ float clip_dist(const f4& v, int k)
{
    switch (k) {
    case 0: return v.w - v.z;
    case 1: return v.z;
    case 2: return GUARD_BAND * v.w + v.x;
    case 3: return GUARD_BAND * v.w - v.x;
    case 4: return GUARD_BAND * v.w + v.y;
    default: return GUARD_BAND * v.w - v.y;
    }
}

__device__ __forceinline__ f4 clip_intersect(const f4& in, const f4& out, float din, float dout)
{
    const float t = din / (din - dout);
    f4 r;
    r.x = in.x + (out.x - in.x) * t;
    r.y = in.y + (out.y - in.y) * t;
    r.z = in.z + (out.z - in.z) * t;
    r.w = in.w + (out.w - in.w) * t;
    return r;
}

#define CLIP_MAXV 10
#define CLIP_THREADS 64u
template <uint32_t STRIDE>
struct ClipLds {
    float4* poly; float* pu; float* pv; int32_t* px; int32_t* py; float* pd; uint32_t tl;
    __device__ __forceinline__ float4& P(int bf, int i) const { return poly[((uint32_t)bf * CLIP_MAXV + (uint32_t)i) * STRIDE + tl]; }
    __device__ __forceinline__ float& U(int bf, int i) const { return pu[((uint32_t)bf * CLIP_MAXV + (uint32_t)i) * STRIDE + tl]; }
    __device__ __forceinline__ float& V(int bf, int i) const { return pv[((uint32_t)bf * CLIP_MAXV + (uint32_t)i) * STRIDE + tl]; }
    __device__ __forceinline__ int32_t& X(int i) const { return px[(uint32_t)i * STRIDE + tl]; }
    __device__ __forceinline__ int32_t& Y(int i) const { return py[(uint32_t)i * STRIDE + tl]; }
    __device__ __forceinline__ float& D(int i) const { return pd[(uint32_t)i * STRIDE + tl]; }
};

template <uint32_t STRIDE>
__device__ __forceinline__ int clip_triangle(const RasterParams& p, const ClipLds<STRIDE>& L, const DMeshlet& m, uint32_t V, uint32_t tri,
                                             const Mat4& mvp, bool masked, int& cur)
{
    const uint32_t packedIdx = p.meshletData[m.dataOffset + V + tri];
    for (int i = 0; i < 3; i++) {
        const uint32_t li = (packedIdx >> (8 * i)) & 0xFFu;
        const uint32_t vi = p.meshletData[m.dataOffset + li] + m.vertexBase;
        const float* pos = p.positions + (size_t)vi * 3;
        const f4 h = mul_mv(mvp, pos[0], pos[1], pos[2], 1.0f);
        L.P(0, i) = make_float4(h.x, h.y, h.z, h.w);
        float u = 0.0f, v = 0.0f;
        if (masked && p.texcoords) { u = p.texcoords[(size_t)vi * 2]; v = p.texcoords[(size_t)vi * 2 + 1]; }
        L.U(0, i) = u; L.V(0, i) = v;
    }
    int np = 3;
    cur = 0;
    for (int pl = p.depthClamp ? 2 : 0; pl < 6 && np >= 3; pl++) {
        int m2 = 0;
        for (int i = 0; i < np; i++) {
            const int j = (i + 1) % np;
            const float4 Pv = L.P(cur, i), Qv = L.P(cur, j);
            const f4 P = {Pv.x, Pv.y, Pv.z, Pv.w}, Q = {Qv.x, Qv.y, Qv.z, Qv.w};
            const float pui = L.U(cur, i), pvi = L.V(cur, i), puj = L.U(cur, j), pvj = L.V(cur, j);
            const float dp = clip_dist(P, pl), dq = clip_dist(Q, pl);
            const bool pin = dp >= 0.0f, qin = dq >= 0.0f;
            if (pin && m2 < CLIP_MAXV) { L.U(cur ^ 1, m2) = pui; L.V(cur ^ 1, m2) = pvi; L.P(cur ^ 1, m2) = Pv; m2++; }
            if (pin && !qin && m2 < CLIP_MAXV) {
                const float t = dp / (dp - dq);
                L.U(cur ^ 1, m2) = pui + (puj - pui) * t; L.V(cur ^ 1, m2) = pvi + (pvj - pvi) * t;
                const f4 x = clip_intersect(P, Q, dp, dq);
                L.P(cur ^ 1, m2) = make_float4(x.x, x.y, x.z, x.w); m2++;
            } else if (!pin && qin && m2 < CLIP_MAXV) {
                const float t = dq / (dq - dp);
                L.U(cur ^ 1, m2) = puj + (pui - puj) * t; L.V(cur ^ 1, m2) = pvj + (pvi - pvj) * t;
                const f4 x = clip_intersect(Q, P, dq, dp);
                L.P(cur ^ 1, m2) = make_float4(x.x, x.y, x.z, x.w); m2++;
            }
        }
        np = m2; cur ^= 1;
    }
    if (np < 3) return 0;
    for (int i = 0; i < np; i++) {
        const float4 h = L.P(cur, i);
        if (!(h.w > 0.0f)) return 0;
        const float u = h.x / fabsf(h.w) * 0.5f + 0.5f;
        const float v = h.y / fabsf(h.w) * -0.5f + 0.5f;
        L.X(i) = (int32_t)rintf((u * p.W) * 256.0f);
        L.Y(i) = (int32_t)rintf((v * p.H) * 256.0f);
        L.D(i) = h.z / h.w;
    }
    return np;
}

__device__ void raster_clip_part(const RasterParams& p, uint32_t block, uint32_t blocks)
{
    __shared__ float4 sPoly[2 * CLIP_MAXV * CLIP_THREADS];
    __shared__ float sPU[2 * CLIP_MAXV * CLIP_THREADS], sPV[2 * CLIP_MAXV * CLIP_THREADS];
    __shared__ int32_t sPX[CLIP_MAXV * CLIP_THREADS], sPY[CLIP_MAXV * CLIP_THREADS];
    __shared__ float sPD[CLIP_MAXV * CLIP_THREADS];
    if (threadIdx.x >= CLIP_THREADS) return;
    const ClipLds<CLIP_THREADS> L = {sPoly, sPU, sPV, sPX, sPY, sPD, threadIdx.x};
    const uint32_t n = min(p.counters->clipTriCount[p.pass], p.clipTriCap);
    const uint32_t listShard = block % CHORD_LIST_SHARDS;
    for (uint32_t k = block * CLIP_THREADS + threadIdx.x; k < n; k += blocks * CLIP_THREADS) {
        const ClipTri ct = p.clipTris[k];
        ChordDrawCmd cmd; cmd.objectId = ct.objectId; cmd.meshletId = ct.meshletId; cmd.slot = ct.slot;
        const DMeshlet& m = p.meshlets[cmd.meshletId];
        const uint32_t V = m.vertexTriangleCount & 0xFFu;
        const uint32_t matFlags = p.objStatic[cmd.objectId].matFlags;
        const bool twoSided = (matFlags & CHORD_MATFLAG_TWO_SIDED) != 0u || p.depthOnly != 0u;
        const bool masked = CHORD_MATFLAG_ALPHA(matFlags) == CHORD_ALPHA_MASK;
        const float* mv = p.objFrame[cmd.objectId].mvp;
        Mat4 mvp;
        for (int r = 0; r < 4; r++) for (int cc = 0; cc < 4; cc++) mvp.r[r][cc] = mv[r * 4 + cc];
        int cur;
        const int np = clip_triangle(p, L, m, V, ct.tri, mvp, masked, cur);
        if (np < 3) continue;
        const uint32_t payload = p.depthOnly ? 0u : encode_triangle_instance(ct.tri, cmd.slot);
        const uint32_t slots = masked ? 1u + CHORD_MASK_EXT_SLOTS : 1u;
        for (int i = 1; i + 1 < np; i++) {
            TriSetup ts;
            ts.X[0] = L.X(0); ts.X[1] = L.X(i); ts.X[2] = L.X(i + 1);
            ts.Y[0] = L.Y(0); ts.Y[1] = L.Y(i); ts.Y[2] = L.Y(i + 1);
            float d[3] = {L.D(0), L.D(i), L.D(i + 1)};
            ts.payload = payload;
            if (!tri_setup(ts, twoSided, p.Wi, p.Hi) || !owns_rect(p.shard, ts.px0, ts.py0, ts.px1, ts.py1)) continue;
            if (p.biasConst != 0.0f || p.biasSlope != 0.0f) { const float o = depth_bias(ts, d, p.biasConst, p.biasSlope); d[0] += o; d[1] += o; d[2] += o; }
            const uint32_t li = atomicAdd(&p.counters->triCount[listShard * CHORD_SHARD_STRIDE], slots);
            if (li + slots > p.triCap) { atomicOr(&p.counters->overflow, 1u); continue; }
            const uint32_t gi = listShard * p.triCap + li;
            write_record(&p.tris[gi], ts, d, twoSided, masked);
            if (masked) {
                const uint32_t material = CHORD_MATFLAG_MATERIAL(matFlags);
                const float u3[3] = {L.U(cur, 0), L.U(cur, i), L.U(cur, i + 1)}, v3[3] = {L.V(cur, 0), L.V(cur, i), L.V(cur, i + 1)};
                const float w3[3] = {L.P(cur, 0).w, L.P(cur, i).w, L.P(cur, i + 1).w};
                write_mask_ext(&p.tris[gi + 1u], &p.materials[material], material, ts.area, u3, v3, w3);
            }
            bin_record_tiles(p, ts, gi | (masked ? CHORD_REC_MASKED : CHORD_REC_WIDE));
        }
    }
}

#define CLIP_BLOCKS 64u
__device__ void raster_bin_large_part(const RasterParams& p, uint32_t block, uint32_t blocks)
{
    const uint32_t lane = threadIdx.x & 63u, wave = threadIdx.x >> 6;
    __shared__ uint32_t sStart[CHORD_LIST_SHARDS + 1];
    if (threadIdx.x < 64u) {
        const uint32_t cnt = min(p.counters->largeCount[p.pass][threadIdx.x * CHORD_SHARD_STRIDE], p.largeCap);
        uint32_t incl = cnt;
#pragma unroll
        for (int d = 1; d < 64; d <<= 1) { const uint32_t nb = (uint32_t)__shfl_up((int)incl, d, 64); if (lane >= (uint32_t)d) incl += nb; }
        sStart[threadIdx.x + 1u] = incl;
        if (threadIdx.x == 0u) sStart[0] = 0u;
    }
    __syncthreads();
    const uint32_t n = sStart[CHORD_LIST_SHARDS];
    for (uint32_t k = block * 4u + wave; k < n; k += blocks * 4u) {
        uint32_t sh = 0;
#pragma unroll
        for (uint32_t st = 32u; st > 0u; st >>= 1) if (sStart[sh + st] <= k) sh += st;
        const uint32_t gi = __builtin_amdgcn_readfirstlane(p.largeList[(size_t)sh * p.largeCap + (k - sStart[sh])]);
        const TriRec* __restrict__ r = &p.tris[gi];
        TriSetup ts;
#pragma unroll
        for (int i = 0; i < 3; i++) { ts.X[i] = r->X[i]; ts.Y[i] = r->Y[i]; }
        ts.payload = 0;
        if (!tri_setup(ts, (r->twoSided & 1u) != 0, p.Wi, p.Hi)) continue;
        const bool maskedRec = (r->twoSided & 4u) != 0u;
        const int ea[3] = {1, 2, 0}, eb[3] = {2, 0, 1};
        int64_t a[3], b[3], bias[3], dxe[3], dye[3];
#pragma unroll
        for (int i = 0; i < 3; i++) {
            dxe[i] = (int64_t)(ts.X[eb[i]] - ts.X[ea[i]]); dye[i] = (int64_t)(ts.Y[eb[i]] - ts.Y[ea[i]]);
            a[i] = -(int64_t)ts.s * dye[i]; b[i] = (int64_t)ts.s * dxe[i];
            bias[i] = (a[i] > 0 || (a[i] == 0 && b[i] > 0)) ? 0 : -1;
        }
        const int32_t tx0 = ts.px0 >> TILE_SHIFT, tx1 = ts.px1 >> TILE_SHIFT;
        const int32_t ty0 = ts.py0 >> TILE_SHIFT, ty1 = ts.py1 >> TILE_SHIFT;
        const uint32_t tw = (uint32_t)(tx1 - tx0 + 1), nt = tw * (uint32_t)(ty1 - ty0 + 1);
        for (uint32_t tb = 0; tb < nt; tb += 64u) {
            const uint32_t t = tb + lane;
            if (t >= nt) continue;
            const int32_t tx = tx0 + (int32_t)(t % tw), ty = ty0 + (int32_t)(t / tw);
            const int32_t rx0 = max(ts.px0, tx << TILE_SHIFT), rx1 = min(ts.px1, (tx << TILE_SHIFT) + TILE - 1);
            const int32_t ry0 = max(ts.py0, ty << TILE_SHIFT), ry1 = min(ts.py1, (ty << TILE_SHIFT) + TILE - 1);
            bool hit = owns_tile(p.shard, tx, ty);
#pragma unroll
            for (int i = 0; i < 3; i++) {
                const int64_t cx = (int64_t)(a[i] > 0 ? rx1 : rx0) * 256 + 128, cy = (int64_t)(b[i] > 0 ? ry1 : ry0) * 256 + 128;
                const int64_t E = (int64_t)ts.s * (dxe[i] * (cy - ts.Y[ea[i]]) - dye[i] * (cx - ts.X[ea[i]]));
                hit = hit && !(E + bias[i] < 0);
            }
            if (hit) {
                const uint32_t tile = (uint32_t)ty * p.tilesX + (uint32_t)tx;
                const uint32_t slot = atomicAdd(&p.tileCount[(size_t)tile * TC_STRIDE], 1u);
                bin_store(p, tile, slot, gi | (maskedRec ? CHORD_REC_MASKED : CHORD_REC_WIDE));
                if (maskedRec) p.tileCount[(size_t)tile * TC_STRIDE + TC_MASKED] = 1u;
            }
        }
    }
}

__global__ __launch_bounds__(256) void raster_clip_and_bin_large_kernel(RasterParams p)
{
    if (blockIdx.x < CLIP_BLOCKS) raster_clip_part(p, blockIdx.x, CLIP_BLOCKS);
    else raster_bin_large_part(p, blockIdx.x - CLIP_BLOCKS, gridDim.x - CLIP_BLOCKS);
}

#define TILE_SLICE_SHIFT CHORD_TILE_SLICE_SHIFT
#define TILE_SLICE (1u << TILE_SLICE_SHIFT)
#ifndef TILE_SPLIT_MIN
#define TILE_SPLIT_MIN 6144u
#endif
#ifndef TILE_ORDER_KEEP
#define TILE_ORDER_KEEP 1
#endif
#ifndef TILE_MAKE_NEXT
#define TILE_MAKE_NEXT 1
#endif
#ifndef TILE_DIRECT
#define TILE_DIRECT 1
#endif
#ifndef TILE_DIRECT_MAX_CLUSTERS
#define TILE_DIRECT_MAX_CLUSTERS 1024u
#endif
#ifndef TILE_SLICE_MIN
#define TILE_SLICE_MIN 1024u
#endif
template <uint32_t NT>
__device__ __forceinline__ void tile_order_part(const RasterParams& p, uint2* __restrict__ order)
{
    __shared__ uint32_t hist[20], base[20], cursor[20], splitItems, splitCursor, longest, hotCount, hotList[CHORD_HOT_TILES], entriesAll, tilesBusy;
    const uint32_t tiles = p.tilesX * p.tilesY;
    if (threadIdx.x < 20u) { hist[threadIdx.x] = 0; cursor[threadIdx.x] = 0; }
    if (threadIdx.x == 0) { splitItems = 0; splitCursor = 0; longest = 0; hotCount = 0; entriesAll = 0; tilesBusy = 0; }
    __syncthreads();
    auto tile_word = [&](uint32_t t) -> uint32_t {
        if (!owns_tile(p.shard, (int32_t)(t % p.tilesX), (int32_t)(t / p.tilesX))) return 0xFFFFFFFFu;
        const uint32_t* __restrict__ line = &p.tileCount[(size_t)t * TC_STRIDE];
        const uint32_t n = line[0], nb = line[1], nm = line[3];
        return min(n, bin_capacity(p)) | (nb ? 0x80000000u : 0u) | (nm ? 0x40000000u : 0u);
    };
    constexpr uint32_t PER_THREAD = CHORD_MAX_TILES / NT;
    uint32_t mine[PER_THREAD];
#pragma unroll
    for (uint32_t k = 0; k < PER_THREAD; k++) { const uint32_t t = threadIdx.x + k * NT; mine[k] = t < tiles ? tile_word(t) : 0xFFFFFFFFu; }
    uint32_t sumMine = 0, tilesMine = 0;
    if (p.tileSlots) {
#pragma unroll
        for (uint32_t k = 0; k < PER_THREAD; k++) {
            const uint32_t w = mine[k];
            if (w != 0xFFFFFFFFu) { const uint32_t c = w & 0x3FFFFFFFu; sumMine += c; tilesMine += c ? 1u : 0u; }
        }
        wave_sum2(sumMine, tilesMine);
        if ((threadIdx.x & 63u) == 0u) { atomicAdd(&entriesAll, sumMine); atomicAdd(&tilesBusy, tilesMine); }
        __syncthreads();
    }
    uint32_t splitMin = p.tileSplitMin, sliceLen = p.tileSliceLen;
    if (p.tileSlots && tilesBusy < p.tileSlots) {
        const uint32_t share = (entriesAll / p.tileSlots + 511u) & ~511u;
        sliceLen = min(p.tileSliceLen, max(TILE_SLICE_MIN, share));
        splitMin = min(p.tileSplitMin, sliceLen + sliceLen / 2u);
    }
    auto slices_of = [&](uint32_t c) -> uint32_t { return (c > splitMin && !ABL(p, DBG_NO_SPLIT)) ? min((c + sliceLen - 1u) / sliceLen, CHORD_TILE_MAX_SLICES) : 0u; };
#pragma unroll
    for (uint32_t k = 0; k < PER_THREAD; k++) {
        const uint32_t t = threadIdx.x + k * NT, w = mine[k];
        if (w == 0xFFFFFFFFu) continue;
        const uint32_t c = w & 0x3FFFFFFFu;
        if (c >= p.slotHot && p.hotTiles) { const uint32_t h = atomicAdd(&hotCount, 1u); if (h < CHORD_HOT_TILES) hotList[h] = t | (c >= SLOT_VERY_HOT ? 0x80000000u : 0u); }
        const uint32_t sl = slices_of(c);
        if (sl) {
            atomicAdd(&splitItems, sl);
            if (c > TILE_SPLIT_MIN) atomicMax(&longest, c);
        } else atomicAdd(&hist[c ? 16u - (31u - (uint32_t)__clz(c)) : 17u], 1u);
    }
    __syncthreads();
    if (threadIdx.x == 0) {
        uint32_t acc = splitItems;
        for (int b = 0; b < 18; b++) { base[b] = acc; acc += hist[b]; }
        order[0] = make_uint2((p.clearTiles || p.orderAll) ? acc : acc - hist[17], 0u);
        if (p.binHint) *p.binHint = longest;
        if (p.heavyHint) p.heavyHint[(splitItems != 0u || *p.count > TILE_DIRECT_MAX_CLUSTERS) ? 0 : 2] = p.binStamp;
        if (p.countHint) *p.countHint = *p.count;
        if (p.hotTiles) p.hotTiles[0] = min(hotCount, (uint32_t)CHORD_HOT_TILES);
    }
    if (p.hotTiles && threadIdx.x < min(hotCount, (uint32_t)CHORD_HOT_TILES)) p.hotTiles[1u + threadIdx.x] = hotList[threadIdx.x];
    __syncthreads();
#pragma unroll
    for (uint32_t k = 0; k < PER_THREAD; k++) {
        const uint32_t t = threadIdx.x + k * NT, w = mine[k];
        if (w == 0xFFFFFFFFu) continue;
        const uint32_t c = w & 0x3FFFFFFFu, sl = slices_of(c);
        if (sl) {
            const uint32_t pos = atomicAdd(&splitCursor, sl);
            for (uint32_t j = 0; j < sl; j++) order[1u + pos + j] = make_uint2(t | (j << 12) | ((sl - 1u) << 22), w);
        } else {
            const uint32_t b = c ? 16u - (31u - (uint32_t)__clz(c)) : 17u;
            order[1u + base[b] + atomicAdd(&cursor[b], 1u)] = make_uint2(t, w);
        }
    }
}

__device__ __noinline__ void tile_order_next_part(const RasterParams* q)
{
    tile_order_part<512u>(*q, q->tileOrderNext);
}

__global__ __launch_bounds__(1024) void raster_tile_order_kernel(RasterParams p)
{
    tile_order_part<1024u>(p, p.tileOrder);
}



struct WideEdges {
    int64_t a[3], b[3], bias[3], dx[3], dy[3];
    int32_t Xa[3], Ya[3];
    int32_t s;
};

__device__ __forceinline__ void wide_edges(const TriSetup& ts, WideEdges& w)
{
    const int ea[3] = {1, 2, 0}, eb[3] = {2, 0, 1};
    w.s = ts.s;
#pragma unroll
    for (int i = 0; i < 3; i++) {
        w.dx[i] = (int64_t)(ts.X[eb[i]] - ts.X[ea[i]]);
        w.dy[i] = (int64_t)(ts.Y[eb[i]] - ts.Y[ea[i]]);
        w.Xa[i] = ts.X[ea[i]]; w.Ya[i] = ts.Y[ea[i]];
        w.a[i] = -(int64_t)ts.s * w.dy[i];
        w.b[i] = (int64_t)ts.s * w.dx[i];
        w.bias[i] = (w.a[i] > 0 || (w.a[i] == 0 && w.b[i] > 0)) ? 0 : -1;
    }
}

__device__ __forceinline__ int64_t edge_at(const WideEdges& w, int i, int32_t px, int32_t py)
{
    const int64_t cx = (int64_t)px * 256 + 128, cy = (int64_t)py * 256 + 128;
    return (int64_t)w.s * (w.dx[i] * (cy - w.Ya[i]) - w.dy[i] * (cx - w.Xa[i]));
}

__device__ __forceinline__ void lds_write(unsigned long long* tile, int32_t lx, int32_t ly, float z, uint32_t payload)
{
    const unsigned long long packed = ((unsigned long long)__float_as_uint(z) << 32) | (unsigned long long)payload;
    atomicMax(&tile[ly * TPITCH + lx], packed);
}

template <int PITCH>
__device__ __forceinline__ void tile_raster_narrow(unsigned long long* tile, const TriSetup& ts, int32_t ox, int32_t oy,
                                                   int32_t x0, int32_t y0, int32_t x1, int32_t y1, bool noPixels, const bool clampZ)
{
    const bool neg = ts.s < 0;
    const int32_t dx0 = ts.X[2] - ts.X[1], dy0 = ts.Y[2] - ts.Y[1];
    const int32_t dx1 = ts.X[0] - ts.X[2], dy1 = ts.Y[0] - ts.Y[2];
    const int32_t dx2 = ts.X[1] - ts.X[0], dy2 = ts.Y[1] - ts.Y[0];
    const int32_t a0 = neg ? dy0 : -dy0, b0 = neg ? -dx0 : dx0;
    const int32_t a1 = neg ? dy1 : -dy1, b1 = neg ? -dx1 : dx1;
    const int32_t a2 = neg ? dy2 : -dy2, b2 = neg ? -dx2 : dx2;
    const int32_t bias0 = (a0 > 0 || (a0 == 0 && b0 > 0)) ? 0 : -1;
    const int32_t bias1 = (a1 > 0 || (a1 == 0 && b1 > 0)) ? 0 : -1;
    const int32_t bias2 = (a2 > 0 || (a2 == 0 && b2 > 0)) ? 0 : -1;
    const int32_t cx0 = x0 * 256 + 128, cy0 = y0 * 256 + 128;
    int32_t r0 = __mul24(b0, cy0 - ts.Y[1]) + __mul24(a0, cx0 - ts.X[1]) + bias0;
    int32_t r1 = __mul24(b1, cy0 - ts.Y[2]) + __mul24(a1, cx0 - ts.X[2]) + bias1;
    int32_t r2 = __mul24(b2, cy0 - ts.Y[0]) + __mul24(a2, cx0 - ts.X[0]) + bias2;
    int32_t E0 = r0, E1 = r1, E2 = r2;
    const int32_t w = x1 - x0 + 1, count = __mul24(w, y1 - y0 + 1);
    const int32_t sx0 = a0 * 256, sx1 = a1 * 256, sx2 = a2 * 256;
    const int32_t sw0 = b0 * 256 - __mul24(w - 1, sx0), sw1 = b1 * 256 - __mul24(w - 1, sx1), sw2 = b2 * 256 - __mul24(w - 1, sx2);
    int32_t col = 0;
    unsigned long long* px = tile + (y0 - oy) * PITCH + (x0 - ox);
    const unsigned long long payload = (unsigned long long)ts.payload;
    for (int32_t i = 0; i < count; i++) {
        const bool inside = (E0 | E1 | E2) >= 0 && !noPixels;
        const float l1 = (float)(E1 - bias1) * ts.invA, l2 = (float)(E2 - bias2) * ts.invA;
        float z = (ts.d0 + l1 * ts.e1) + l2 * ts.e2;
        if (clampZ) z = fminf(fmaxf(z, 0.0f), 1.0f);
        atomicMax(px, inside ? (((unsigned long long)__float_as_uint(z) << 32) | payload) : 0ull);
        col++;
        const bool wrap = col == w;
        E0 += wrap ? sw0 : sx0; E1 += wrap ? sw1 : sx1; E2 += wrap ? sw2 : sx2;
        px += wrap ? PITCH - w + 1 : 1;
        col = wrap ? 0 : col;
    }
}

#ifndef TINY_AREA
#define TINY_AREA 8
#endif
#ifndef TINY_AREA_DENSE
#define TINY_AREA_DENSE 48
#endif
#ifndef TINY_DENSE_MIN
#define TINY_DENSE_MIN 1024u
#endif

struct UnitParams {
    int32_t X[3], Y[3];
    float d0, e1, e2, invA;
    uint32_t payload;
    uint32_t box;
    int32_t skind;
};
#define TB 512
static_assert(TB == 512, "tile_order_part rounds a pass's slice length to batches of 512");
#define UNIT_CAP 4096

template <typename E_t>
__device__ __forceinline__ void scan_row(unsigned long long* __restrict__ tileRow, const UnitParams& u, int32_t ox, int32_t py,
                                         int32_t lx0, int32_t lx1, bool noPixels, const bool clampZ)
{
    const E_t s = (u.skind & 1) ? (E_t)-1 : (E_t)1;
    const E_t dx0 = (E_t)(u.X[2] - u.X[1]), dy0 = (E_t)(u.Y[2] - u.Y[1]);
    const E_t dx1 = (E_t)(u.X[0] - u.X[2]), dy1 = (E_t)(u.Y[0] - u.Y[2]);
    const E_t dx2 = (E_t)(u.X[1] - u.X[0]), dy2 = (E_t)(u.Y[1] - u.Y[0]);
    const E_t a0 = -s * dy0, b0 = s * dx0, a1 = -s * dy1, b1 = s * dx1, a2 = -s * dy2, b2 = s * dx2;
    const E_t bias0 = (a0 > 0 || (a0 == 0 && b0 > 0)) ? (E_t)0 : (E_t)-1;
    const E_t bias1 = (a1 > 0 || (a1 == 0 && b1 > 0)) ? (E_t)0 : (E_t)-1;
    const E_t bias2 = (a2 > 0 || (a2 == 0 && b2 > 0)) ? (E_t)0 : (E_t)-1;
    const E_t cx = (E_t)(ox + lx0) * (E_t)256 + (E_t)128, cy = (E_t)py * (E_t)256 + (E_t)128;
    E_t E0 = s * (dx0 * (cy - (E_t)u.Y[1]) - dy0 * (cx - (E_t)u.X[1])) + bias0;
    E_t E1 = s * (dx1 * (cy - (E_t)u.Y[2]) - dy1 * (cx - (E_t)u.X[2])) + bias1;
    E_t E2 = s * (dx2 * (cy - (E_t)u.Y[0]) - dy2 * (cx - (E_t)u.X[0])) + bias2;
    const E_t st0 = a0 * (E_t)256, st1 = a1 * (E_t)256, st2 = a2 * (E_t)256;
    float klo = 0.0f, khi = (float)(lx1 - lx0);
    {
        const float e[3] = {(float)E0, (float)E1, (float)E2}, t[3] = {(float)st0, (float)st1, (float)st2};
#pragma unroll
        for (int i = 0; i < 3; i++) {
            const float q = fminf(fmaxf(-e[i] * __builtin_amdgcn_rcpf(t[i]), -4.0f), 4096.0f);
            if (t[i] > 0.0f) klo = fmaxf(klo, floorf(q) - 1.0f);
            else if (t[i] < 0.0f) khi = fminf(khi, floorf(q) + 1.0f);
            else if (e[i] < 0.0f) khi = -1.0f;
        }
    }
    const int32_t k0 = (int32_t)klo, k1 = (int32_t)khi;
    E0 += (E_t)k0 * st0; E1 += (E_t)k0 * st1; E2 += (E_t)k0 * st2;
    unsigned long long* px = tileRow + lx0 + k0;
    const unsigned long long payload = noPixels ? 0ull : (unsigned long long)u.payload;
    for (int32_t k = k0; k <= k1; k++) {
// ... 810 lines not shown
                uint32_t seg = nseg == 1u ? 0u : nseg == 2u ? (j & 1u) : nseg == 4u ? (j & 3u) : j % 3u;
                for (uint32_t u = lo2; u < hi2; u++) {
                    unitList[u - r0] = tix | (row << 9) | (seg << 15);
                    if (++seg == nseg) { seg = 0u; row++; }
                }
            }
        };
        for (uint32_t r0 = 0; r0 < total; r0 += TILE_UNIT_CAP) {
            list_units(offN, rowsN, r0);
            __syncthreads();
            const uint32_t nr = min(total - r0, (uint32_t)TILE_UNIT_CAP);
            for (uint32_t ui = tix; ui < nr; ui += TB) {
                const uint32_t d = unitList[ui];
                if (ABL(p, DBG_NO_UNITS)) continue;
                const int32_t trips = entry_unit<MASKED, DEPTH>(p, prm, tile, d & 511u, (d >> 9) & 63u, (d >> 15) & 3u, ox, oy, noPixels);
                if (prof) { cUnits++; cUnitIters += (uint32_t)trips; }
            }
            if (r0 + TILE_UNIT_CAP < total || totalM) __syncthreads();
        }
        for (uint32_t r0 = 0; r0 < totalM; r0 += TILE_UNIT_CAP) {
            if (rowsM) {
                const uint32_t box = prm.w[11][tix];
                const uint32_t nseg = ((((box >> 12) & 63u) - (box & 63u)) >> MASKED_SEG_SHIFT) + 1u, y0l = (box >> 6) & 63u;
                const uint32_t lo2 = max(offM, r0), hi2 = min(offM + rowsM, r0 + TILE_UNIT_CAP);
                if (lo2 < hi2) {
                    const uint32_t j = lo2 - offM, g = j / nseg;
                    uint32_t row = y0l + g * MASKED_ROWS, seg = j - g * nseg;
                    for (uint32_t u = lo2; u < hi2; u++) {
                        unitList[u - r0] = tix | (row << 9) | (seg << 15);
                        if (++seg == nseg) { seg = 0u; row += MASKED_ROWS; }
                    }
                }
            }
            __syncthreads();
            const uint32_t nr = min(totalM - r0, (uint32_t)TILE_UNIT_CAP);
            for (uint32_t ui = tix; ui < nr; ui += TB) {
                const uint32_t d = unitList[ui];
                entry_unit_masked<DEPTH>(p, prm, tile, d & 511u, (d >> 9) & 63u, (d >> 15) & 7u, ox, oy, noPixels);
            }
            if (r0 + TILE_UNIT_CAP < totalM) __syncthreads();
        }
        total |= totalM;
        if (total) __syncthreads();
        PHASE(4);
    };
    uint32_t batchNo = 0;
    if constexpr (TILE_DEEP_FETCH && !MASKED) {
        uint32_t nameA = nameNext, nameB = idxNext;
        uint4 b0 = make_uint4(0, 0, 0, 0), b1 = b0, b2 = b0;
        if (nameB != 0xFFFFFFFFu) FETCH_REC(nameB, b0, b1, b2);
        uint32_t idx = entryThread && k0 + 2u * TILE_BATCH < n ? binEntry(k0 + 2u * TILE_BATCH) : 0xFFFFFFFFu;
        for (uint32_t base = lo; base < n;) {
            window_advance(base);
            uint32_t rows = batch_setup(nq0, nq1, nq2, nameA);
            nameA = idx;
            if (nameA != 0xFFFFFFFFu) FETCH_REC(nameA, nq0, nq1, nq2);
            idx = entryThread && base + tix + 3u * TILE_BATCH < n ? binEntry(base + tix + 3u * TILE_BATCH) : 0xFFFFFFFFu;
            batch_units(rows, batchNo);
            base += TILE_BATCH; batchNo++;
            if (base >= n) break;
            window_advance(base);
            rows = batch_setup(b0, b1, b2, nameB);
            nameB = idx;
            if (nameB != 0xFFFFFFFFu) FETCH_REC(nameB, b0, b1, b2);
            idx = entryThread && base + tix + 3u * TILE_BATCH < n ? binEntry(base + tix + 3u * TILE_BATCH) : 0xFFFFFFFFu;
            batch_units(rows, batchNo);
            base += TILE_BATCH; batchNo++;
        }
    } else
    for (uint32_t base = lo; base < n; base += TILE_BATCH, batchNo++) {
        window_advance(base);
        const uint32_t k = base + tix;
        const uint4 q0 = nq0, q1 = nq1, q2 = nq2;
        const uint32_t name = nameNext;
        nameNext = idxNext;
        if (nameNext != 0xFFFFFFFFu) FETCH_REC(nameNext, nq0, nq1, nq2);
        idxNext = entryThread && k + 2u * TILE_BATCH < n ? binEntry(k + 2u * TILE_BATCH) : 0xFFFFFFFFu;
        batch_units(batch_setup(q0, q1, q2, name), batchNo);
    }
    __syncthreads();

    if (mergeSlices) {
        const RasterParams* q = kernel_args();
        if (!merge_slices(tile, scalar_load(&q->tileSlabs) + (size_t)tileId * (TILE * TILE), &scalar_load(&q->tileCount)[(size_t)tileId * TC_STRIDE + TC_TICKET],
                          slices, &sTicket, &scalar_load(&q->counters)->overflow)) continue;
        if (rmw) {
            for (uint32_t i = tix, visBase = vis_base(); i < TILE * TILE / 2; i += TB) {
                const int32_t ly = (int32_t)(i >> (TILE_SHIFT - 1)), lx = (int32_t)(i & (TILE / 2 - 1)) * 2;
                if (ly >= th || lx >= tw) continue;
                const unsigned long long* src = p.vis + (size_t)(visBase + (uint32_t)ly * visPitch + (uint32_t)lx);
                tile[ly * TPITCH + lx] = max(tile[ly * TPITCH + lx], src[0]);
                if (lx + 1 < tw) tile[ly * TPITCH + lx + 1] = max(tile[ly * TPITCH + lx + 1], src[1]);
            }
        }
        __syncthreads();
    }

    if (ABL(p, DBG_NO_OUT)) {
    } else if (p.hzbFused && !ABL(p, DBG_NO_HZB)) {
        tile_out_and_hzb<SH>(tile, reinterpret_cast<float*>(&prm.w[0][0]), offs, tileId, slot_of_tile(), nAll, ox, oy, tw, th);
    } else if (p.clearTiles || p.hzbFused) {
        for (uint32_t i = tix, visBase = vis_base(); i < TILE * TILE / 2; i += TB) {
            const int32_t ly = (int32_t)(i >> (TILE_SHIFT - 1)), lx = (int32_t)(i & (TILE / 2 - 1)) * 2;
            if (ly >= th || lx >= tw) continue;
            const ulonglong2 v = make_ulonglong2(tile[ly * TPITCH + lx], tile[ly * TPITCH + lx + 1]);
            unsigned long long* dst = p.vis + (size_t)(visBase + (uint32_t)ly * visPitch + (uint32_t)lx);
            if (lx + 1 < tw) *reinterpret_cast<ulonglong2*>(dst) = v;
            else dst[0] = v.x;
        }
    } else {
        for (uint32_t i = tix, visBase = vis_base(); i < TILE * TILE; i += TB) {
            const int32_t ly = (int32_t)(i >> TILE_SHIFT), lx = (int32_t)(i & (TILE - 1));
            const unsigned long long v = tile[ly * TPITCH + lx];
            if (v != 0ull && ly < th && lx < tw) atomicMax(p.vis + (size_t)(visBase + (uint32_t)ly * visPitch + (uint32_t)lx), v);
        }
    }
    PHASE(5);
    if (prof) {
        if (tix == 0) {
            p.tileClocks[tileId] = wall_clock64() - t0;
            for (int i = 0; i < 6; i++) p.tilePhase[(size_t)tileId * 8 + i] = ph[i];
            p.tilePhase[(size_t)tileId * 8 + 6] = 0ull; p.tilePhase[(size_t)tileId * 8 + 7] = 0ull;
        }
        __syncthreads();
        atomicAdd(&p.tilePhase[(size_t)tileId * 8 + 6], ((unsigned long long)cUnits << 32) | cUnitIters);
        atomicAdd(&p.tilePhase[(size_t)tileId * 8 + 7], ((unsigned long long)cTiny << 32) | cTinyIters);
        if ((tix & 63u) == 0u) for (int i = 0; i < 6; i++) atomicAdd(&p.tilePhase[(size_t)tileId * 8 + i], bw[i] << 32);
    }
    __syncthreads();
    }
}
#undef wgs
#undef TILE_SKEW

#if !CHORD_MASKED_FUSED && TILE_BATCH != TB
#error "the separate masked pass sets up one entry per thread of its workgroup: TILE_BATCH must be TB"
#endif
#if TILE_BATCH == TB
template <bool SH, bool DEPTH>
__global__ __launch_bounds__(TB, 4) void raster_masked_tile_kernel(RasterParams p)
{
    __shared__ __align__(16) unsigned long long tile[TILE * TPITCH];
    __shared__ EntrySoA prm;
    __shared__ uint32_t unitList[UNIT_CAP];
    __shared__ uint32_t waveSums[2][TB / 64];
    __shared__ uint32_t chunkTab[64];
    const uint32_t active = p.tileOrder[0].x;
    for (uint32_t oi = blockIdx.x; oi < active; oi += gridDim.x) {
    const uint2 item = p.tileOrder[1u + oi];
    if ((item.y & 0x40000000u) == 0u || ((item.x >> 12) & 0x3FFu) != 0u) continue;
    const uint32_t tileId = item.x & 0xFFFu;
    const uint32_t n = item.y & 0x3FFFFFFFu;
    const int32_t ox = (int32_t)(tileId % p.tilesX) * TILE, oy = (int32_t)(tileId / p.tilesX) * TILE;
    const int32_t tw = min(TILE, p.Wi - ox), th = min(TILE, p.Hi - oy);
    const bool noPixels = ABL(p, DBG_NO_PIXELS);
    for (uint32_t i = threadIdx.x; i < TILE * TPITCH / 2; i += TB) reinterpret_cast<ulonglong2*>(tile)[i] = make_ulonglong2(0ull, 0ull);
    const uint32_t* bin = p.tileBins + (size_t)tileId * p.binCap;
    const uint32_t wideLimit = min(p.triCap * CHORD_LIST_SHARDS, CHORD_REC_WIDE_INDEX);
    uint32_t batch = 0;
    for (uint32_t segLo = 0; segLo < n;) {
        uint32_t segHi, chunk0 = 0;
        if (segLo < p.binCap) segHi = min(n, p.binCap);
        else {
            chunk0 = (segLo - p.binCap) >> CHORD_BIN_CHUNK_SHIFT;
            segHi = min(n, segLo + 64u * CHORD_BIN_CHUNK);
            __syncthreads();
            for (uint32_t j = threadIdx.x; j < 64u; j += TB) {
                const unsigned long long e = chunk0 + j < p.binMaxChunks ? p.binChunkTab[(size_t)tileId * p.binMaxChunks + chunk0 + j] : 0ull;
                chunkTab[j] = (uint32_t)(e >> 32) == p.binStamp ? (uint32_t)e : CHORD_BIN_CHUNK_INVALID;
            }
        }
        __syncthreads();
        auto binWord = [&](uint32_t k) -> uint32_t {
            if (k < p.binCap) return bin[k];
            const uint32_t o = k - p.binCap, cj = (o >> CHORD_BIN_CHUNK_SHIFT) - chunk0;
            const uint32_t id = cj < 64u ? chunkTab[cj] : CHORD_BIN_CHUNK_INVALID;
            return id == CHORD_BIN_CHUNK_INVALID ? 0xFFFFFFFFu : p.binPool[(size_t)id * CHORD_BIN_CHUNK + (o & (CHORD_BIN_CHUNK - 1u))];
        };
        uint32_t wNext = segLo + threadIdx.x < segHi ? binWord(segLo + threadIdx.x) : 0xFFFFFFFFu;
        for (uint32_t base = segLo; base < segHi; base += TB, batch++) {
            const uint32_t w = wNext;
            wNext = base + TB + threadIdx.x < segHi ? binWord(base + TB + threadIdx.x) : 0xFFFFFFFFu;
            const uint32_t idx = w & CHORD_REC_WIDE_INDEX;
            uint32_t units = 0;
            if ((w & 0xE0000000u) == CHORD_REC_MASKED && idx < wideLimit) {
                const uint4* src = reinterpret_cast<const uint4*>(&p.tris[idx]);
                const uint4 q0 = src[0], q1 = src[1], q2 = src[2];
                TriRec r;
                r.X[0] = (int32_t)q0.x; r.X[1] = (int32_t)q0.y; r.X[2] = (int32_t)q0.z; r.Y[0] = (int32_t)q0.w;
                r.Y[1] = (int32_t)q1.x; r.Y[2] = (int32_t)q1.y;
                r.d[0] = __uint_as_float(q1.z); r.d[1] = __uint_as_float(q1.w); r.d[2] = __uint_as_float(q2.x);
                r.payload = q2.y; r.twoSided = q2.z; r.pad = q2.w;
                TriSetup ts;
                tri_setup_from_record(ts, r, p.Wi, p.Hi);
                const int32_t x0 = max(ts.px0, ox), y0 = max(ts.py0, oy);
                const int32_t x1 = min(ts.px1, ox + tw - 1), y1 = min(ts.py1, oy + th - 1);
                if (x1 >= x0 && y1 >= y0) units = entry_store(prm, threadIdx.x, ts, narrow_extent(ts), ox, oy, x0, y0, x1, y1, true, idx);
            }
            uint32_t total;
            const uint32_t off = block_scan_tb(units, waveSums[batch & 1u], &total);
            for (uint32_t r0 = 0; r0 < total; r0 += UNIT_CAP) {
                if (units) {
                    const uint32_t box = prm.w[11][threadIdx.x];
                    const uint32_t nseg = ((((box >> 12) & 63u) - (box & 63u)) >> MASKED_SEG_SHIFT) + 1u, y0l = (box >> 6) & 63u;
                    const uint32_t lo2 = max(off, r0), hi2 = min(off + units, r0 + UNIT_CAP);
                    if (lo2 < hi2) {
                        const uint32_t j = lo2 - off, g = j / nseg;
                        uint32_t row = y0l + g * MASKED_ROWS, seg = j - g * nseg;
                        for (uint32_t u = lo2; u < hi2; u++) {
                            unitList[u - r0] = threadIdx.x | (row << 9) | (seg << 15);
                            if (++seg == nseg) { seg = 0u; row += MASKED_ROWS; }
                        }
                    }
                }
                __syncthreads();
                const uint32_t nr = min(total - r0, (uint32_t)UNIT_CAP);
                for (uint32_t ui = threadIdx.x; ui < nr; ui += TB) {
                    const uint32_t d = unitList[ui];
                    entry_unit_masked<DEPTH>(p, prm, tile, d & 511u, (d >> 9) & 63u, (d >> 15) & 7u, ox, oy, noPixels);
                }
                if (r0 + UNIT_CAP < total) __syncthreads();
            }
            if (total) __syncthreads();
        }
        segLo = segHi;
    }
    __syncthreads();
    const uint32_t visBase = SH ? p.shard.tileSlot[tileId] << (2 * TILE_SHIFT) : (uint32_t)oy * (uint32_t)p.Wi + (uint32_t)ox;
    const uint32_t visPitch = SH ? (uint32_t)TILE : (uint32_t)p.Wi;
    if (p.clearTiles) {
        for (uint32_t i = threadIdx.x; i < TILE * TILE / 2; i += TB) {
            const int32_t ly = (int32_t)(i >> (TILE_SHIFT - 1)), lx = (int32_t)(i & (TILE / 2 - 1)) * 2;
            if (ly >= th || lx >= tw) continue;
            const ulonglong2 v = make_ulonglong2(tile[ly * TPITCH + lx], tile[ly * TPITCH + lx + 1]);
            unsigned long long* dst = p.vis + (size_t)(visBase + (uint32_t)ly * visPitch + (uint32_t)lx);
            if (lx + 1 < tw) *reinterpret_cast<ulonglong2*>(dst) = v;
            else dst[0] = v.x;
        }
    } else {
        for (uint32_t i = threadIdx.x; i < TILE * TILE; i += TB) {
            const int32_t ly = (int32_t)(i >> TILE_SHIFT), lx = (int32_t)(i & (TILE - 1));
            const unsigned long long v = tile[ly * TPITCH + lx];
            if (v != 0ull && ly < th && lx < tw) atomicMax(p.vis + (size_t)(visBase + (uint32_t)ly * visPitch + (uint32_t)lx), v);
        }
    }
    __syncthreads();
    }
}
#endif

hipError_t launch_raster(ChordCtx* c, const CmdList& in, bool clearTiles)
{
#define LR_HIP(call) do { const hipError_t e_ = (call); if (e_ != hipSuccess) return e_; } while (0)
    RasterParams p;
    p.hzbFused = 0; p.hzbMinA = nullptr; p.hzbMinB = nullptr; p.hzbMaxB = nullptr; p.tileRange = c->dTileRange;
    p.hzbExA = nullptr; p.hzbExB = nullptr;
    p.hzbDesc = c->hzb[0].desc;
    if (c->fuseHzb && c->shard.ranks == 1) {
        p.hzbFused = 1;
        p.hzbMinA = (clearTiles && c->fuseHzbTemp) ? c->hzb[0].minTexels : nullptr;
        p.hzbMinB = c->hzb[c->fuseHzbSlot].minTexels; p.hzbMaxB = c->hzb[c->fuseHzbSlot].maxTexels;
    } else if (c->fuseHzb) {
        p.hzbFused = 1;
        p.hzbExA = (clearTiles && c->fuseHzbTemp) ? c->dHzbExchange : nullptr;
        p.hzbExB = c->dHzbFinalExchange;
    }
    p.count = in.count; p.cmds = in.cmds; p.cmdCap = std::max(in.capacity, 1u);
    if (c->shard.ranks > 1) {
        bool mine = false;
        if (in.cmds == c->lists[0].cmds && c->mineValid) { p.count = c->dCounts + 4; p.cmds = c->dMineCmds; mine = true; }
        else if (in.cmds == c->dMineCmds && c->mineValid) mine = true;
        else for (int k = 1; k < 3; k++) if (in.cmds == c->lists[k].cmds && c->listMine[k]) mine = true;
        if (!mine) {
            if (!c->dRankCmds) LR_HIP(hipMalloc((void**)&c->dRankCmds, sizeof(ChordDrawCmd) * (size_t)c->cmdCapacity));
            CmdList filtered;
            filtered.count = c->dCounts + 5; filtered.cmds = c->dRankCmds; filtered.capacity = in.capacity;
            LR_HIP(hipMemsetAsync(filtered.count, 0, sizeof(uint32_t), c->stream));
            launch_rank_filter(c, in, filtered);
            p.count = filtered.count; p.cmds = filtered.cmds;
        }
    }
    p.objFrame = c->dObjFrame; p.objStatic = c->dObjStatic;
    p.meshlets = c->dMeshlets; p.meshletData = c->dMeshletData; p.positions = c->dPositions;
    p.materials = c->dMaterials; p.texAlpha = c->dTexAlpha; p.texcoords = c->dTexcoords;
    p.vis = (unsigned long long*)c->dVis;
    p.depthOut = (p.hzbFused && clearTiles) ? c->depthOutTarget : nullptr;
    p.W = (float)c->width; p.H = (float)c->height; p.Wi = (int32_t)c->width; p.Hi = (int32_t)c->height;
    p.shard = c->shard;
    p.blockPool = c->dBlockPool; p.blockCap = (c->debugFlags & DBG_NO_BLOCKS) ? 0u : c->blockCap;
    p.blockForce = (c->debugFlags & DBG_FORCE_BLOCKS) ? 1u : 0u;
    p.tris = c->dTris; p.triCap = c->triCap / CHORD_LIST_SHARDS;
    p.trisC = c->dTrisC; p.triCapC = c->triCapC / CHORD_LIST_SHARDS;
    const uint32_t tiles = c->tilesX * c->tilesY;
    const uint32_t pass = c->rasterCalls & 1u;
    p.tileCount = c->dFrameState->tileCount + (size_t)pass * tiles * TC_STRIDE;
    p.tileBins = c->dTileBins + (size_t)pass * tiles * c->binCap; p.binCap = c->binCap;
    p.binPool = c->dBinPool + (size_t)pass * c->binPoolChunks * CHORD_BIN_CHUNK; p.binPoolChunks = c->binPoolChunks;
    p.binPoolCount = &c->dCounters->binPoolCount[pass];
    p.binChunkTab = c->dBinChunkTab + (size_t)pass * tiles * c->binMaxChunks; p.binMaxChunks = c->binMaxChunks;
    p.binStamp = ++c->rasterSerial;
    p.tilesX = c->tilesX; p.tilesY = c->tilesY;
    p.clipTris = c->dClipTris + (size_t)pass * (c->clipTriCap / 2); p.clipTriCap = c->clipTriCap / 2; p.pass = pass;
    p.largeList = c->dLargeList + (size_t)pass * (c->largeCap / 2); p.largeCap = c->largeCap / 2 / CHORD_LIST_SHARDS;
    p.counters = c->dCounters;
    p.clearTiles = clearTiles ? 1u : 0u;
    p.depthOnly = c->depthOnly ? 1u : 0u; p.depthClamp = c->depthClamp ? 1u : 0u;
    p.biasConst = c->depthBiasConst; p.biasSlope = c->depthBiasSlope;
    p.debug = c->debugFlags;
    p.tileClocks = c->dTileClocks + (size_t)pass * CHORD_MAX_TILES;
    p.tileOrder = reinterpret_cast<uint2*>(c->dTileOrder); p.tileSlabs = c->dTileSlabs;
    p.tilePhase = c->dTileClocks + (size_t)2 * CHORD_MAX_TILES + (size_t)pass * CHORD_MAX_TILES * 8;

    if (!c->inFrame || c->rasterCalls >= 2) {
        LR_HIP(hipMemsetAsync(p.tileCount, 0, sizeof(uint32_t) * TC_STRIDE * tiles, c->stream));
        LR_HIP(hipMemsetAsync(&c->dCounters->clipTriCount[pass], 0, sizeof(uint32_t), c->stream));
        LR_HIP(hipMemsetAsync(c->dCounters->largeCount[pass], 0, sizeof(c->dCounters->largeCount[pass]), c->stream));
        LR_HIP(hipMemsetAsync(&c->dCounters->binPoolCount[pass], 0, sizeof(uint32_t), c->stream));
        if (!c->inFrame) { LR_HIP(hipMemsetAsync(c->dCounters->triCount, 0, sizeof(c->dCounters->triCount), c->stream));
                           LR_HIP(hipMemsetAsync(c->dCounters->triCountC, 0, sizeof(c->dCounters->triCountC), c->stream));
                           LR_HIP(hipMemsetAsync(c->dCounters->blockGranules, 0, sizeof(c->dCounters->blockGranules), c->stream)); }
    }

    const uint64_t rankPixels = (uint64_t)c->width * c->height / (c->shard.ranks > 1 ? c->shard.ranks : 1u);
    const bool maybeDense = p.blockCap != 0u && (p.blockForce != 0u || (uint64_t)in.capacity * 16ull >= rankPixels);
    p.leftCount = nullptr; p.leftCmds = nullptr;
    p.binHint = nullptr; p.countHint = nullptr;
    p.slotHot = (c->debugFlags & DBG_FORCE_HOT) ? 64u : SLOT_HOT;
    {
        static const int forced = [] { const char* e = getenv("CHORDVIS_TILE_SLOTS"); return e ? atoi(e) : -1; }();
        p.tileSlots = forced >= 0 ? (uint32_t)forced : c->shard.ranks > 1 ? (uint32_t)c->numCUs * (CHORD_TILE_SHIFT == 6 ? 2u : 6u) : 0u;
        static const int splitMin = [] { const char* e = getenv("CHORDVIS_TILE_SPLIT_MIN"); return e ? atoi(e) : -1; }();
        static const int sliceLen = [] { const char* e = getenv("CHORDVIS_TILE_SLICE"); return e ? atoi(e) : -1; }();
        p.tileSplitMin = splitMin > 0 ? (uint32_t)splitMin : TILE_SPLIT_MIN;
        p.tileSliceLen = sliceLen >= 512 ? ((uint32_t)sliceLen + 511u) & ~511u : TILE_SLICE;
    }
    p.hotTiles = c->dHotTiles ? c->dHotTiles + (size_t)pass * (1u + CHORD_HOT_TILES) : nullptr;
    bool blocksWorthLaunching = maybeDense;
    if (maybeDense && c->dBinHint) {
        p.countHint = c->dBinHint + 2 + pass;
        const uint32_t last = c->hBinHint[2 + pass];
        if (p.blockForce == 0u && last != 0xFFFFFFFFu && (uint64_t)last * 32ull < rankPixels) blocksWorthLaunching = false;
    }
    if (blocksWorthLaunching) {
        if (c->dBinHint) p.binHint = c->dBinHint + pass;
        if (!c->dLeftCmds) LR_HIP(hipMalloc((void**)&c->dLeftCmds, sizeof(ChordDrawCmd) * (size_t)c->cmdCapacity));
        p.leftCount = c->dCounts + 6 + pass; p.leftCmds = c->dLeftCmds;
        if (!c->inFrame || c->rasterCalls >= 2) LR_HIP(hipMemsetAsync(p.leftCount, 0, sizeof(uint32_t), c->stream));
    }
    p.orderKept = 0u;
    p.heavyHint = nullptr;
    static const bool directOn = [] { const char* e = getenv("CHORDVIS_TILE_DIRECT"); return !e || atoi(e) != 0; }();
    const bool laterOk = c->inFrame && !clearTiles && p.hzbFused && !c->depthOnly && CHORD_MASKED_FUSED && c->dBinHint && !(c->debugFlags & ~(DBG_NO_BLOCKS | DBG_FORCE_BLOCKS | DBG_FORCE_HOT | 524288u));
    if (laterOk) p.heavyHint = c->dBinHint + 4 + pass;
    if (TILE_DIRECT && directOn && laterOk) {
        const uint32_t heavySeen = c->hBinHint[4 + pass], lightSeen = c->hBinHint[6 + pass];
        if (lightSeen != 0u && (heavySeen == 0u || (int32_t)(lightSeen - heavySeen) > 0)) {
            p.orderKept = 2u;
        }
    }
    static const int touchedEnv = [] { const char* e = getenv("CHORDVIS_TILE_TOUCHED"); return e ? atoi(e) : 1; }();
    p.tileTouched = nullptr;
    if (p.orderKept == 2u && touchedEnv != 0 && c->shard.ranks <= 1 && tiles <= 64u * 64u) {
        p.tileTouched = c->dFrameState->tileTouched + (size_t)pass * (CHORD_MAX_TILES / 32u);
        if (!c->inFrame || c->rasterCalls >= 2) LR_HIP(hipMemsetAsync(p.tileTouched, 0, sizeof(uint32_t) * ((tiles + 31u) / 32u), c->stream));
    }
    uint32_t blocks = (in.capacity + 3u) / 4u;
#ifndef SETUP_GRID_MULT
#define SETUP_GRID_MULT 1u
#endif
    const uint32_t maxBlocks = (uint32_t)c->numCUs * SETUP_MIN_WAVES * SETUP_GRID_MULT;
    if (blocks > maxBlocks) blocks = maxBlocks;
    if (blocks < 1) blocks = 1;
    const bool sh = c->shard.ranks > 1;
    stamp(c, S_HZBCULL);
    if (blocksWorthLaunching) {
        const uint32_t bb = std::max(1u, std::min((in.capacity + 3u) / 4u, (uint32_t)c->numCUs * BLOCKS_MIN_WAVES));
        const bool hot = (c->hBinHint && c->hBinHint[pass] >= SLOT_HOT) || (c->debugFlags & DBG_FORCE_HOT);
        if (hot) CHORD_LAUNCH(c, raster_setup_blocks_kernel<true>, dim3(bb), dim3(256), 0, c->stream, p);
        else     CHORD_LAUNCH(c, raster_setup_blocks_kernel<false>, dim3(bb), dim3(256), 0, c->stream, p);
    }
    if (c->anyMasked) CHORD_LAUNCH(c, raster_setup_kernel<true>, dim3(blocks), dim3(256), 0, c->stream, p);
    else              CHORD_LAUNCH(c, raster_setup_kernel<false>, dim3(blocks), dim3(256), 0, c->stream, p);
    stamp(c, S_R_CLUSTER);
    CHORD_LAUNCH(c, raster_clip_and_bin_large_kernel, dim3(CLIP_BLOCKS + (uint32_t)c->numCUs * 4u), dim3(256), 0, c->stream, p);
    bool makeOrder = p.orderKept != 2u;
    p.orderAll = 0u; p.tileOrderNext = nullptr;
    static const bool keepLaterOn = [] { const char* e = getenv("CHORDVIS_TILE_KEEP_LATER"); return !e || atoi(e) != 0; }();
    static const bool nextOn = [] { const char* e = getenv("CHORDVIS_TILE_NEXT"); return !e || atoi(e) != 0; }();
    const bool keepOk = TILE_ORDER_KEEP && c->orderKeepFrames && CHORD_MASKED_FUSED && c->inFrame && !c->depthOnly && !(c->debugFlags & ~524288u);
    int slot = -1;
    if (keepOk && clearTiles && pass == 0u && c->dTileOrderKeep) slot = 0;
    else if (keepOk && keepLaterOn && laterOk && pass == 1u && c->dTileOrderKeep1) slot = 1;
    if (slot >= 0) {
        uint32_t& age = slot ? c->orderAge1 : c->orderAge;
        uint2* buf = reinterpret_cast<uint2*>(slot ? c->dTileOrderKeep1 : c->dTileOrderKeep);
        const size_t half = (size_t)1 + c->tileItemCap;
        p.orderAll = slot ? 1u : 0u;
        if (nextOn && p.orderKept == 2u) {
            age = 0xFFFFFFFFu; p.orderAll = 0u;
        } else if (nextOn) {
            uint32_t& flip = c->orderFlip[slot];
            p.tileOrder = buf + flip * half; p.tileOrderNext = buf + (flip ^ 1u) * half;
            if (age != 0xFFFFFFFFu) { p.orderKept = 1u; makeOrder = false; }
            age = 0u; flip ^= 1u;
        } else if (p.orderKept != 2u) {
            p.tileOrder = buf;
            if (age < c->orderKeepFrames) { age++; p.orderKept = 1u; makeOrder = false; }
            else age = 0u;
        } else p.orderAll = 0u;
    }
    if (makeOrder) CHORD_LAUNCH(c, raster_tile_order_kernel, dim3(1), dim3(1024), 0, c->stream, p);
#if !CHORD_MASKED_FUSED
    if (c->anyMasked) {
        const uint32_t items = tiles;
        if (c->depthClamp && !sh) CHORD_LAUNCH(c, (raster_masked_tile_kernel<false, true>), dim3(items), dim3(TB), 0, c->stream, p);
        else if (sh)              CHORD_LAUNCH(c, (raster_masked_tile_kernel<true, false>), dim3(items), dim3(TB), 0, c->stream, p);
        else                      CHORD_LAUNCH(c, (raster_masked_tile_kernel<false, false>), dim3(items), dim3(TB), 0, c->stream, p);
    }
#endif
    stamp(c, S_R_CLIP);
    const uint32_t slots = (uint32_t)c->numCUs * (CHORD_TILE_SHIFT == 6 ? 2u : 6u);
    const uint32_t tileBlocks = (p.tileOrderNext ? 1u : 0u) + ((clearTiles || (p.orderKept == 2u && !p.tileTouched) || p.orderAll) ? ((sh && clearTiles) ? min(tiles, max(c->shard.slotsPerRank, p.tileSlots + p.tileSlots / 2u)) : tiles)
                                                               : min(tiles, p.tileTouched && touchedEnv > 1 ? (uint32_t)touchedEnv : slots));
#if CHORD_MASKED_FUSED
    if (c->anyMasked) {
        if (c->depthClamp && !sh) CHORD_LAUNCH(c, (raster_tile_kernel<false, true, true>), dim3(tileBlocks), dim3(TB), 0, c->stream, p);
        else if (sh)              CHORD_LAUNCH(c, (raster_tile_kernel<true, true, false>), dim3(tileBlocks), dim3(TB), 0, c->stream, p);
        else                      CHORD_LAUNCH(c, (raster_tile_kernel<false, true, false>), dim3(tileBlocks), dim3(TB), 0, c->stream, p);
    } else
#endif
    if (c->depthClamp && !sh) {
        CHORD_LAUNCH(c, (raster_tile_kernel<false, false, true>), dim3(tileBlocks), dim3(TB), 0, c->stream, p);
    } else {
        if (sh) CHORD_LAUNCH(c, (raster_tile_kernel<true, false, false>), dim3(tileBlocks), dim3(TB), 0, c->stream, p);
        else    CHORD_LAUNCH(c, (raster_tile_kernel<false, false, false>), dim3(tileBlocks), dim3(TB), 0, c->stream, p);
    }
    stamp(c, S_R_CHUNK);
    c->rasterCalls++;
    return hipSuccess;
#undef LR_HIP
}

}
```

Baseline: 3.276 Gtri/s.

## Fold large-triangle binning and clipping into the setup kernel

Moves large-triangle tile binning and near/guard-band clipping out of the separate clip-and-bin-large kernel and into the raster setup kernel. Setup waves stage large triangles in LDS and distribute their tile tests across lanes, and they clip triangles inline using slices of the vertex LDS. The intent is to remove a kernel launch and the global round trip through the large and clip lists. In exchange, setup carries more LDS use and register pressure, and some lanes do divergent clipping work. An env var can restore the old path.

```diff
diff --git a/chord_amd/csrc/kernels_raster.hip b/chord_amd/csrc/kernels_raster.hip
--- a/chord_amd/csrc/kernels_raster.hip
+++ b/chord_amd/csrc/kernels_raster.hip
@@ -43,6 +43,7 @@
     uint32_t blockForce;
     ClipTri* clipTris; uint32_t clipTriCap; uint32_t pass;
     uint32_t* largeList; uint32_t largeCap;
+    uint32_t binInSetup;
     DeviceCounters* counters;
     uint2* tileOrder;
     unsigned long long* tileSlabs;
@@ -247,6 +248,7 @@
     uint32_t* binPool; uint32_t binPoolChunks; uint32_t* binPoolCount;
     unsigned long long* binChunkTab; uint32_t binStamp; uint32_t binMaxChunks;
     uint32_t* tileTouched;
+    uint32_t binInSetup;
     ShardInfo shard;
 };
 __device__ __forceinline__ RecordEmitParams load_record_emit_params()
@@ -259,7 +261,7 @@
     e.tileCount = scalar_load(&q->tileCount); e.tileBins = scalar_load(&q->tileBins); e.binCap = scalar_load(&q->binCap); e.tilesX = scalar_load(&q->tilesX);
     e.binPool = scalar_load(&q->binPool); e.binPoolChunks = scalar_load(&q->binPoolChunks); e.binPoolCount = scalar_load(&q->binPoolCount);
     e.binChunkTab = scalar_load(&q->binChunkTab); e.binStamp = scalar_load(&q->binStamp); e.binMaxChunks = scalar_load(&q->binMaxChunks);
-    e.tileTouched = scalar_load(&q->tileTouched);
+    e.tileTouched = scalar_load(&q->tileTouched); e.binInSetup = scalar_load(&q->binInSetup);
     e.shard.ranks = scalar_load(&q->shard.ranks); e.shard.rank = scalar_load(&q->shard.rank); e.shard.slotsPerRank = 0u; e.shard.tilesX = 0u;
     e.shard.ownedRows = scalar_load(&q->shard.ownedRows); e.shard.tileSlot = nullptr;
     return e;
@@ -323,7 +325,8 @@
     if (id != CHORD_BIN_CHUNK_INVALID) p.binPool[((size_t)id << CHORD_BIN_CHUNK_SHIFT) + (o & (CHORD_BIN_CHUNK - 1u))] = gi;
 }
 
-__device__ __forceinline__ void bin_store(const RasterParams& p, uint32_t tile, uint32_t slot, uint32_t gi)
+template <class P>
+__device__ __forceinline__ void bin_store(const P& p, uint32_t tile, uint32_t slot, uint32_t gi)
 {
     bin_alloc(p, tile, slot);
     bin_put(p, tile, slot, gi);
@@ -598,6 +601,264 @@
     a = (uint32_t)__builtin_amdgcn_readlane((int)a, 63); b = (uint32_t)__builtin_amdgcn_readlane((int)b, 63);
 }
 
+template <class P>
+__device__ __forceinline__ void bin_record_tiles(const P& p, const TriSetup& ts, uint32_t gi)
+{
+    const int ea[3] = {1, 2, 0}, eb[3] = {2, 0, 1};
+    const int32_t tx0 = ts.px0 >> TILE_SHIFT, tx1 = ts.px1 >> TILE_SHIFT;
+    const int32_t ty0 = ts.py0 >> TILE_SHIFT, ty1 = ts.py1 >> TILE_SHIFT;
+    for (int32_t ty = ty0; ty <= ty1; ty++)
+        for (int32_t tx = tx0; tx <= tx1; tx++) {
+            const int32_t rx0 = max(ts.px0, tx << TILE_SHIFT), rx1 = min(ts.px1, (tx << TILE_SHIFT) + TILE - 1);
+            const int32_t ry0 = max(ts.py0, ty << TILE_SHIFT), ry1 = min(ts.py1, (ty << TILE_SHIFT) + TILE - 1);
+            bool hit = owns_tile(p.shard, tx, ty);
+#pragma unroll
+            for (int i = 0; i < 3; i++) {
+                const int64_t dxe = (int64_t)(ts.X[eb[i]] - ts.X[ea[i]]), dye = (int64_t)(ts.Y[eb[i]] - ts.Y[ea[i]]);
+                const int64_t a = -(int64_t)ts.s * dye, b = (int64_t)ts.s * dxe;
+                const int64_t bias = (a > 0 || (a == 0 && b > 0)) ? 0 : -1;
+                const int64_t cx = (int64_t)(a > 0 ? rx1 : rx0) * 256 + 128, cy = (int64_t)(b > 0 ? ry1 : ry0) * 256 + 128;
+                hit = hit && !((int64_t)ts.s * (dxe * (cy - ts.Y[ea[i]]) - dye * (cx - ts.X[ea[i]])) + bias < 0);
+            }
+            if (!hit) continue;
+            const uint32_t tile = (uint32_t)ty * p.tilesX + (uint32_t)tx;
+            const uint32_t slot = atomicAdd(&p.tileCount[(size_t)tile * TC_STRIDE], 1u);
+            bin_store(p, tile, slot, gi);
+            if ((gi & 0xE0000000u) == CHORD_REC_MASKED) p.tileCount[(size_t)tile * TC_STRIDE + TC_MASKED] = 1u;
+        }
+}
+
+#define LARGE_ROUND 1
+struct LargeLds {
+    float* f[5];
+    __device__ __forceinline__ uint32_t& at(int field, uint32_t k) const { return reinterpret_cast<uint32_t*>(f[field >> 1])[(uint32_t)(field & 1) * 128u + k]; }
+};
+enum { LG_X0 = 0, LG_Y0 = 3, LG_S = 6, LG_BX = 7, LG_BY = 8, LG_GI = 9 };
+__device__ __forceinline__ void large_put(const LargeLds& L, uint32_t k, const TriSetup& ts)
+{
+#pragma unroll
+    for (int i = 0; i < 3; i++) { L.at(LG_X0 + i, k) = (uint32_t)ts.X[i]; L.at(LG_Y0 + i, k) = (uint32_t)ts.Y[i]; }
+    L.at(LG_S, k) = (uint32_t)ts.s;
+    L.at(LG_BX, k) = (uint32_t)ts.px0 | (uint32_t)ts.px1 << 16; L.at(LG_BY, k) = (uint32_t)ts.py0 | (uint32_t)ts.py1 << 16;
+}
+__device__ __forceinline__ uint32_t large_tiles(uint32_t bx, uint32_t by)
+{
+    return (((bx >> 16) >> TILE_SHIFT) - ((bx & 0xFFFFu) >> TILE_SHIFT) + 1u) * (((by >> 16) >> TILE_SHIFT) - ((by & 0xFFFFu) >> TILE_SHIFT) + 1u);
+}
+template <class P>
+__device__ __forceinline__ void wave_bin_large(const P& e, const LargeLds& L, bool hasA, bool hasB, uint32_t lane)
+{
+    const uint32_t nA = hasA ? large_tiles(L.at(LG_BX, lane), L.at(LG_BY, lane)) : 0u;
+    const uint32_t n = nA + (hasB ? large_tiles(L.at(LG_BX, 64u + lane), L.at(LG_BY, 64u + lane)) : 0u);
+    uint32_t incl = n;
+#pragma unroll
+    for (int d = 1; d < 64; d <<= 1) { const uint32_t nb = (uint32_t)__shfl_up((int)incl, d, 64); if (lane >= (uint32_t)d) incl += nb; }
+    const uint32_t total = bcast(incl, 63), excl = incl - n;
+    for (uint32_t base = 0; base < total; base += 64u * LARGE_ROUND) {
+        uint32_t tile[LARGE_ROUND], slot[LARGE_ROUND], gi[LARGE_ROUND];
+        bool hit[LARGE_ROUND];
+#pragma unroll
+        for (int r = 0; r < LARGE_ROUND; r++) {
+            const uint32_t j = base + (uint32_t)r * 64u + lane, jj = min(j, total - 1u);
+            int src = 0;
+#pragma unroll
+            for (int st = 32; st > 0; st >>= 1) if ((uint32_t)__shfl((int)incl, src + st - 1, 64) <= jj) src += st;
+            const uint32_t off = jj - (uint32_t)__shfl((int)excl, src, 64), offA = (uint32_t)__shfl((int)nA, src, 64);
+            const uint32_t k = (uint32_t)src + (off >= offA ? 64u : 0u), t = off >= offA ? off - offA : off;
+            TriSetup ts;
+#pragma unroll
+            for (int i = 0; i < 3; i++) { ts.X[i] = (int32_t)L.at(LG_X0 + i, k); ts.Y[i] = (int32_t)L.at(LG_Y0 + i, k); }
+            ts.s = (int32_t)L.at(LG_S, k);
+            const uint32_t bx = L.at(LG_BX, k), by = L.at(LG_BY, k);
+            gi[r] = L.at(LG_GI, k);
+            ts.px0 = (int32_t)(bx & 0xFFFFu); ts.px1 = (int32_t)(bx >> 16); ts.py0 = (int32_t)(by & 0xFFFFu); ts.py1 = (int32_t)(by >> 16);
+            const int32_t tx0 = ts.px0 >> TILE_SHIFT, ty0 = ts.py0 >> TILE_SHIFT;
+            const uint32_t tw = (uint32_t)((ts.px1 >> TILE_SHIFT) - tx0 + 1);
+            const int32_t tx = tx0 + (int32_t)(t % tw), ty = ty0 + (int32_t)(t / tw);
+            const int32_t rx0 = max(ts.px0, tx << TILE_SHIFT), rx1 = min(ts.px1, (tx << TILE_SHIFT) + TILE - 1);
+            const int32_t ry0 = max(ts.py0, ty << TILE_SHIFT), ry1 = min(ts.py1, (ty << TILE_SHIFT) + TILE - 1);
+            const int ea[3] = {1, 2, 0}, eb[3] = {2, 0, 1};
+            bool h = j < total && owns_tile(e.shard, tx, ty);
+#pragma unroll
+            for (int i = 0; i < 3; i++) {
+                const int64_t dxe = (int64_t)(ts.X[eb[i]] - ts.X[ea[i]]), dye = (int64_t)(ts.Y[eb[i]] - ts.Y[ea[i]]);
+                const int64_t a = -(int64_t)ts.s * dye, b = (int64_t)ts.s * dxe;
+                const int64_t bias = (a > 0 || (a == 0 && b > 0)) ? 0 : -1;
+                const int64_t cx = (int64_t)(a > 0 ? rx1 : rx0) * 256 + 128, cy = (int64_t)(b > 0 ? ry1 : ry0) * 256 + 128;
+                h = h && !((int64_t)ts.s * (dxe * (cy - ts.Y[ea[i]]) - dye * (cx - ts.X[ea[i]])) + bias < 0);
+            }
+            hit[r] = h;
+            tile[r] = h ? (uint32_t)ty * e.tilesX + (uint32_t)tx : 0u;
+            slot[r] = h ? atomicAdd(&e.tileCount[(size_t)tile[r] * TC_STRIDE], 1u) : 0u;
+        }
+#pragma unroll
+        for (int r = 0; r < LARGE_ROUND; r++) if (hit[r]) bin_alloc(e, tile[r], slot[r]);
+#pragma unroll
+        for (int r = 0; r < LARGE_ROUND; r++) {
+            if (!hit[r]) continue;
+            bin_put(e, tile[r], slot[r], gi[r]);
+            if ((gi[r] & 0xE0000000u) == CHORD_REC_MASKED) e.tileCount[(size_t)tile[r] * TC_STRIDE + TC_MASKED] = 1u;
+        }
+    }
+}
+
+__device__ __forceinline__ float clip_dist(const f4& v, int k)
+{
+    switch (k) {
+    case 0: return v.w - v.z;
+    case 1: return v.z;
+    case 2: return GUARD_BAND * v.w + v.x;
+    case 3: return GUARD_BAND * v.w - v.x;
+    case 4: return GUARD_BAND * v.w + v.y;
+    default: return GUARD_BAND * v.w - v.y;
+    }
+}
+
+__device__ __forceinline__ f4 clip_intersect(const f4& in, const f4& out, float din, float dout)
+{
+    const float t = din / (din - dout);
+    f4 r;
+    r.x = in.x + (out.x - in.x) * t;
+    r.y = in.y + (out.y - in.y) * t;
+    r.z = in.z + (out.z - in.z) * t;
+    r.w = in.w + (out.w - in.w) * t;
+    return r;
+}
+
+#define CLIP_MAXV 10
+#define CLIP_THREADS 64u
+template <uint32_t STRIDE>
+struct ClipLds {
+    float4* poly; float* pu; float* pv; int32_t* px; int32_t* py; float* pd; uint32_t tl;
+    __device__ __forceinline__ float4& P(int bf, int i) const { return poly[((uint32_t)bf * CLIP_MAXV + (uint32_t)i) * STRIDE + tl]; }
+    __device__ __forceinline__ float& U(int bf, int i) const { return pu[((uint32_t)bf * CLIP_MAXV + (uint32_t)i) * STRIDE + tl]; }
+    __device__ __forceinline__ float& V(int bf, int i) const { return pv[((uint32_t)bf * CLIP_MAXV + (uint32_t)i) * STRIDE + tl]; }
+    __device__ __forceinline__ int32_t& X(int i) const { return px[(uint32_t)i * STRIDE + tl]; }
+    __device__ __forceinline__ int32_t& Y(int i) const { return py[(uint32_t)i * STRIDE + tl]; }
+    __device__ __forceinline__ float& D(int i) const { return pd[(uint32_t)i * STRIDE + tl]; }
+};
+
+template <uint32_t STRIDE, class Prm>
+__device__ __forceinline__ int clip_triangle(const Prm& p, const ClipLds<STRIDE>& L, uint32_t dataOffset, uint32_t vertexBase, uint32_t V, uint32_t tri,
+                                             const Mat4& mvp, bool masked, int& cur)
+{
+    const uint32_t packedIdx = p.meshletData[dataOffset + V + tri];
+    for (int i = 0; i < 3; i++) {
+        const uint32_t li = (packedIdx >> (8 * i)) & 0xFFu;
+        const uint32_t vi = p.meshletData[dataOffset + li] + vertexBase;
+        const float* pos = p.positions + (size_t)vi * 3;
+        const f4 h = mul_mv(mvp, pos[0], pos[1], pos[2], 1.0f);
+        L.P(0, i) = make_float4(h.x, h.y, h.z, h.w);
+        float u = 0.0f, v = 0.0f;
+        if (masked && p.texcoords) { u = p.texcoords[(size_t)vi * 2]; v = p.texcoords[(size_t)vi * 2 + 1]; }
+        L.U(0, i) = u; L.V(0, i) = v;
+    }
+    int np = 3;
+    cur = 0;
+    for (int pl = p.depthClamp ? 2 : 0; pl < 6 && np >= 3; pl++) {
+        int m2 = 0;
+        for (int i = 0; i < np; i++) {
+            const int j = (i + 1) % np;
+            const float4 Pv = L.P(cur, i), Qv = L.P(cur, j);
+            const f4 P = {Pv.x, Pv.y, Pv.z, Pv.w}, Q = {Qv.x, Qv.y, Qv.z, Qv.w};
+            const float pui = L.U(cur, i), pvi = L.V(cur, i), puj = L.U(cur, j), pvj = L.V(cur, j);
+            const float dp = clip_dist(P, pl), dq = clip_dist(Q, pl);
+            const bool pin = dp >= 0.0f, qin = dq >= 0.0f;
+            if (pin && m2 < CLIP_MAXV) { L.U(cur ^ 1, m2) = pui; L.V(cur ^ 1, m2) = pvi; L.P(cur ^ 1, m2) = Pv; m2++; }
+            if (pin && !qin && m2 < CLIP_MAXV) {
+                const float t = dp / (dp - dq);
+                L.U(cur ^ 1, m2) = pui + (puj - pui) * t; L.V(cur ^ 1, m2) = pvi + (pvj - pvi) * t;
+                const f4 x = clip_intersect(P, Q, dp, dq);
+                L.P(cur ^ 1, m2) = make_float4(x.x, x.y, x.z, x.w); m2++;
+            } else if (!pin && qin && m2 < CLIP_MAXV) {
+                const float t = dq / (dq - dp);
+                L.U(cur ^ 1, m2) = puj + (pui - puj) * t; L.V(cur ^ 1, m2) = pvj + (pvi - pvj) * t;
+                const f4 x = clip_intersect(Q, P, dq, dp);
+                L.P(cur ^ 1, m2) = make_float4(x.x, x.y, x.z, x.w); m2++;
+            }
+        }
+        np = m2; cur ^= 1;
+    }
+    if (np < 3) return 0;
+    for (int i = 0; i < np; i++) {
+        const float4 h = L.P(cur, i);
+        if (!(h.w > 0.0f)) return 0;
+        const float u = h.x / fabsf(h.w) * 0.5f + 0.5f;
+        const float v = h.y / fabsf(h.w) * -0.5f + 0.5f;
+        L.X(i) = (int32_t)rintf((u * p.W) * 256.0f);
+        L.Y(i) = (int32_t)rintf((v * p.H) * 256.0f);
+        L.D(i) = h.z / h.w;
+    }
+    return np;
+}
+
+template <uint32_t STRIDE, class P>
+__device__ __forceinline__ void clip_emit(const P& p, const ClipLds<STRIDE>& L, int np, int cur, uint32_t payload, bool twoSided, bool masked,
+                                          uint32_t matFlags, uint32_t listShard)
+{
+    const uint32_t slots = masked ? 1u + CHORD_MASK_EXT_SLOTS : 1u;
+    for (int i = 1; i + 1 < np; i++) {
+        TriSetup ts;
+        ts.X[0] = L.X(0); ts.X[1] = L.X(i); ts.X[2] = L.X(i + 1);
+        ts.Y[0] = L.Y(0); ts.Y[1] = L.Y(i); ts.Y[2] = L.Y(i + 1);
+        float d[3] = {L.D(0), L.D(i), L.D(i + 1)};
+        ts.payload = payload;
+        if (!tri_setup(ts, twoSided, p.Wi, p.Hi) || !owns_rect(p.shard, ts.px0, ts.py0, ts.px1, ts.py1)) continue;
+        if (p.biasConst != 0.0f || p.biasSlope != 0.0f) { const float o = depth_bias(ts, d, p.biasConst, p.biasSlope); d[0] += o; d[1] += o; d[2] += o; }
+        const uint32_t li = atomicAdd(&p.counters->triCount[listShard * CHORD_SHARD_STRIDE], slots);
+        if (li + slots > p.triCap) { atomicOr(&p.counters->overflow, 1u); continue; }
+        const uint32_t gi = listShard * p.triCap + li;
+        write_record(&p.tris[gi], ts, d, twoSided, masked);
+        if (masked) {
+            const uint32_t material = CHORD_MATFLAG_MATERIAL(matFlags);
+            const float u3[3] = {L.U(cur, 0), L.U(cur, i), L.U(cur, i + 1)}, v3[3] = {L.V(cur, 0), L.V(cur, i), L.V(cur, i + 1)};
+            const float w3[3] = {L.P(cur, 0).w, L.P(cur, i).w, L.P(cur, i + 1).w};
+            write_mask_ext(&p.tris[gi + 1u], &p.materials[material], material, ts.area, u3, v3, w3);
+        }
+        bin_record_tiles(p, ts, gi | (masked ? CHORD_REC_MASKED : CHORD_REC_WIDE));
+    }
+}
+
+template <bool MASKED, uint32_t STRIDE, class P>
+__device__ __forceinline__ void clip_entry(const P& p, const ClipLds<STRIDE>& L, const ClipTri ct, uint32_t listShard)
+{
+    const DMeshlet& m = p.meshlets[ct.meshletId];
+    const uint32_t V = m.vertexTriangleCount & 0xFFu;
+    const uint32_t matFlags = p.objStatic[ct.objectId].matFlags;
+    const bool twoSided = (matFlags & CHORD_MATFLAG_TWO_SIDED) != 0u || p.depthOnly != 0u;
+    const bool masked = MASKED && CHORD_MATFLAG_ALPHA(matFlags) == CHORD_ALPHA_MASK;
+    const float* mv = p.objFrame[ct.objectId].mvp;
+    Mat4 mvp;
+    for (int r = 0; r < 4; r++) for (int cc = 0; cc < 4; cc++) mvp.r[r][cc] = mv[r * 4 + cc];
+    int cur;
+    const int np = clip_triangle(p, L, m.dataOffset, m.vertexBase, V, ct.tri, mvp, masked, cur);
+    if (np < 3) return;
+    const uint32_t payload = p.depthOnly ? 0u : encode_triangle_instance(ct.tri, ct.slot);
+    clip_emit(p, L, np, cur, payload, twoSided, masked, matFlags, listShard);
+}
+
+struct SetupClipParams : RecordEmitParams {
+    const DObjFrame* objFrame; const DObjStatic* objStatic; const DMeshlet* meshlets;
+    const uint32_t* meshletData; const float* positions; const float* texcoords; const DMaterial* materials;
+    uint32_t depthOnly; float W, H; int32_t Wi, Hi; uint32_t depthClamp; float biasConst, biasSlope;
+};
+__device__ __forceinline__ SetupClipParams load_setup_clip_params()
+{
+    const RasterParams* q = kernel_args();
+    SetupClipParams c;
+    static_cast<RecordEmitParams&>(c) = load_record_emit_params();
+    c.objFrame = scalar_load(&q->objFrame); c.objStatic = scalar_load(&q->objStatic); c.meshlets = scalar_load(&q->meshlets); c.depthOnly = scalar_load(&q->depthOnly);
+    c.meshletData = scalar_load(&q->meshletData); c.positions = scalar_load(&q->positions); c.texcoords = scalar_load(&q->texcoords);
+    c.materials = scalar_load(&q->materials);
+    c.W = scalar_load(&q->W); c.H = scalar_load(&q->H); c.Wi = scalar_load(&q->Wi); c.Hi = scalar_load(&q->Hi);
+    c.depthClamp = scalar_load(&q->depthClamp); c.biasConst = scalar_load(&q->biasConst); c.biasSlope = scalar_load(&q->biasSlope);
+    return c;
+}
+#define CLIP_SETUP_LANES 3u
+#define CLIP_RANGES 255u
+static_assert(2u * CLIP_MAXV * CLIP_SETUP_LANES * 4u <= LDS_VERTS && 4u * CLIP_MAXV * CLIP_SETUP_LANES <= LDS_VERTS && 3u * CLIP_MAXV * CLIP_SETUP_LANES <= LDS_VERTS,
+              "a set-up wave's clip polygons fit its slices of sVert");
+
 enum { K_NONE = 0, K_EMIT = 1, K_CLIP = 2 };
 #define WIN CHORD_BLOCK_WIN
 #define DBG_NO_BLOCKS 32768u
@@ -605,7 +866,7 @@
 #define DBG_FORCE_HOT 262144u
 
 template <bool MASKED>
-__device__ __forceinline__ void raster_setup_body(const RasterParams& p, const ChordDrawCmd* __restrict__ cmds, const uint32_t count, float (*sVert)[4][LDS_VERTS],
+__device__ __forceinline__ void raster_setup_body(const RasterParams& p, const ChordDrawCmd* __restrict__ cmds, const uint32_t count, float (*sVert)[4][LDS_VERTS], uint32_t* sClip,
                                                   const uint32_t firstCmd0, const uint32_t firstCmd1, const uint32_t firstCmd2, const bool firstCmdValid)
 {
     const uint32_t lane = threadIdx.x & 63u, wave = threadIdx.x >> 6;
@@ -669,6 +930,7 @@
     unsigned long long sph[5] = {0, 0, 0, 0, 0}, stp = sprof ? wall_clock64() : 0ull;
 #define SPHASE(i) do { if (sprof) { const unsigned long long tn = wall_clock64(); sph[i] += tn - stp; stp = tn; } } while (0)
     const uint32_t laneTop = lane;
+    if (lane == 0u) sClip[0] = 0u;
     for (; c < count; c += stride) {
         uint32_t lane = laneTop;
         asm volatile("" : "+v"(lane));
@@ -796,8 +1058,17 @@
             BinTicket ticket;
             if (emA | emB) wave_bin_issue(e, kindA == K_EMIT && !lgA, tsA, kindB == K_EMIT && !lgB, tsB, lane, ticket, MASKED && masked);
             cbase = bcast(cbase, 0); ebaseC = bcast(ebaseC, 0); ebaseW = bcast(ebaseW, 0); lbase = bcast(lbase, 0);
+            if (e.binInSetup && (lmA | lmB)) {
+                const LargeLds LL = {{lX, lY, lU, lV, lD}};
+                if (lgA) large_put(LL, lane, tsA);
+                if (lgB) large_put(LL, 64u + lane, tsB);
+            }
             SPHASE(3);
             mvpNext = mvp_of(hdrN.objectId);
+            if (e.binInSetup && nClip && lane == 0u) {
+                const uint32_t r = sClip[0];
+                if (r < CLIP_RANGES) { sClip[1u + r] = cbase | (nClip - 1u) << 25; sClip[0] = r + 1u; } else atomicOr(&e.counters->overflow, 2u);
+            }
             if (kindA == K_CLIP) {
                 const uint32_t k = cbase + (uint32_t)__popcll(cmA & lt);
                 if (k < e.clipTriCap) { ClipTri ct; ct.objectId = hdr.objectId; ct.meshletId = hdr.meshletId; ct.slot = hdr.slot; ct.tri = lane; e.clipTris[k] = ct; }
@@ -834,12 +1105,19 @@
                     giB |= (MASKED && masked) ? CHORD_REC_MASKED : CHORD_REC_WIDE; okB = true;
                 } else atomicOr(&e.counters->overflow, 1u);
             }
+            const LargeLds LL = {{lX, lY, lU, lV, lD}};
+            if (e.binInSetup && (lmA | lmB)) {
+                if (lgA && okA) LL.at(LG_GI, lane) = giA;
+                if (lgB && okB) LL.at(LG_GI, 64u + lane) = giB;
+            }
             if (emA | emB) wave_bin_commit(e, ticket, okA, giA, okB, giB);
-            if (lgA && okA) {
+            if (e.binInSetup) {
+                if (lmA | lmB) wave_bin_large(e, LL, lgA && okA, lgB && okB, lane);
+            } else if (lgA && okA) {
                 const uint32_t k = lbase + (uint32_t)__popcll(lmA & lt);
                 if (k < e.largeCap) e.largeList[(size_t)listShard * e.largeCap + k] = giA & CHORD_REC_WIDE_INDEX; else atomicOr(&e.counters->overflow, 1u);
             }
-            if (lgB && okB) {
+            if (lgB && okB && !e.binInSetup) {
                 const uint32_t k = lbase + (uint32_t)__popcll(lmA) + (uint32_t)__popcll(lmB & lt);
                 if (k < e.largeCap) e.largeList[(size_t)listShard * e.largeCap + k] = giB & CHORD_REC_WIDE_INDEX; else atomicOr(&e.counters->overflow, 1u);
             }
@@ -852,6 +1130,20 @@
         t0 = nt0; t1 = nt1;
         pax = nax; pay = nay; paz = naz; pbx = nbx; pby = nby; pbz = nbz;
         SPHASE(4);
+    }
+    __builtin_amdgcn_fence(__ATOMIC_RELEASE, "wavefront");
+    __builtin_amdgcn_wave_barrier();
+    __builtin_amdgcn_fence(__ATOMIC_ACQUIRE, "wavefront");
+    if (const uint32_t ranges = __builtin_amdgcn_readfirstlane(sClip[0])) {
+        const SetupClipParams q = load_setup_clip_params();
+        const ClipLds<CLIP_SETUP_LANES> L = {reinterpret_cast<float4*>(lX), lY, lY + 2u * CLIP_MAXV * CLIP_SETUP_LANES,
+                                             reinterpret_cast<int32_t*>(lW), reinterpret_cast<int32_t*>(lW) + CLIP_MAXV * CLIP_SETUP_LANES,
+                                             lW + 2u * CLIP_MAXV * CLIP_SETUP_LANES, lane};
+        for (uint32_t i = 0; i < ranges; i++) {
+            const uint32_t w = __builtin_amdgcn_readfirstlane(sClip[1u + i]), base = w & 0x1FFFFFFu, n = (w >> 25) + 1u;
+            for (uint32_t k0 = 0; k0 < n; k0 += CLIP_SETUP_LANES)
+                if (lane < CLIP_SETUP_LANES && k0 + lane < n && base + k0 + lane < q.clipTriCap) clip_entry<MASKED>(q, L, q.clipTris[base + k0 + lane], listShard);
+        }
     }
     if (sprof && lane == 0u) {
         const uint32_t w = blockIdx.x * 4u + wave;
@@ -1233,7 +1525,8 @@
 template <bool MASKED>
 __global__ __launch_bounds__(256, MASKED ? SETUP_MASKED_WAVES : SETUP_MIN_WAVES) void raster_setup_kernel(RasterParams p)
 {
-    __shared__ float sVert[6][4][LDS_VERTS];
+    __shared__ __attribute__((aligned(16))) float sVert[6][4][LDS_VERTS];
+    __shared__ uint32_t sClip[4][1 + CLIP_RANGES];
     const uint32_t c0 = __builtin_amdgcn_readfirstlane(min(blockIdx.x * 4u + (threadIdx.x >> 6), p.cmdCap - 1u));
     const uint32_t* __restrict__ cw = reinterpret_cast<const uint32_t*>(p.cmds + c0);
     const uint32_t f0 = scalar_load(cw), f1 = scalar_load(cw + 1), f2 = scalar_load(cw + 2);
@@ -1241,7 +1534,7 @@
     const ChordDrawCmd* cmds = p.cmds;
     bool firstValid = true;
     if (launch_is_dense(p, count)) { count = *p.leftCount; cmds = p.leftCmds; firstValid = false; }
-    raster_setup_body<MASKED>(p, cmds, count, sVert, f0, f1, f2, firstValid);
+    raster_setup_body<MASKED>(p, cmds, count, sVert, sClip[threadIdx.x >> 6], f0, f1, f2, firstValid);
 }
 
 template <bool HOT>
@@ -1254,122 +1547,6 @@
     const uint32_t count = *p.count;
     if (!launch_is_dense(p, count)) return;
     raster_setup_blocks_body<HOT>(p, count, sVert, sSnap, sWin, sSlots);
-}
-
-__device__ void bin_record_tiles(const RasterParams& p, const TriSetup& ts, uint32_t gi)
-{
-    const int ea[3] = {1, 2, 0}, eb[3] = {2, 0, 1};
-    const int32_t tx0 = ts.px0 >> TILE_SHIFT, tx1 = ts.px1 >> TILE_SHIFT;
-    const int32_t ty0 = ts.py0 >> TILE_SHIFT, ty1 = ts.py1 >> TILE_SHIFT;
-    for (int32_t ty = ty0; ty <= ty1; ty++)
-        for (int32_t tx = tx0; tx <= tx1; tx++) {
-            const int32_t rx0 = max(ts.px0, tx << TILE_SHIFT), rx1 = min(ts.px1, (tx << TILE_SHIFT) + TILE - 1);
-            const int32_t ry0 = max(ts.py0, ty << TILE_SHIFT), ry1 = min(ts.py1, (ty << TILE_SHIFT) + TILE - 1);
-            bool hit = owns_tile(p.shard, tx, ty);
-#pragma unroll
-            for (int i = 0; i < 3; i++) {
-                const int64_t dxe = (int64_t)(ts.X[eb[i]] - ts.X[ea[i]]), dye = (int64_t)(ts.Y[eb[i]] - ts.Y[ea[i]]);
-                const int64_t a = -(int64_t)ts.s * dye, b = (int64_t)ts.s * dxe;
-                const int64_t bias = (a > 0 || (a == 0 && b > 0)) ? 0 : -1;
-                const int64_t cx = (int64_t)(a > 0 ? rx1 : rx0) * 256 + 128, cy = (int64_t)(b > 0 ? ry1 : ry0) * 256 + 128;
-                hit = hit && !((int64_t)ts.s * (dxe * (cy - ts.Y[ea[i]]) - dye * (cx - ts.X[ea[i]])) + bias < 0);
-            }
-            if (!hit) continue;
-            const uint32_t tile = (uint32_t)ty * p.tilesX + (uint32_t)tx;
-            const uint32_t slot = atomicAdd(&p.tileCount[(size_t)tile * TC_STRIDE], 1u);
-            bin_store(p, tile, slot, gi);
-            if ((gi & 0xE0000000u) == CHORD_REC_MASKED) p.tileCount[(size_t)tile * TC_STRIDE + TC_MASKED] = 1u;
-        }
-}
-
-__device__ __forceinline__ float clip_dist(const f4& v, int k)
-{
-    switch (k) {
-    case 0: return v.w - v.z;
-    case 1: return v.z;
-    case 2: return GUARD_BAND * v.w + v.x;
-    case 3: return GUARD_BAND * v.w - v.x;
-    case 4: return GUARD_BAND * v.w + v.y;
-    default: return GUARD_BAND * v.w - v.y;
-    }
-}
-
-__device__ __forceinline__ f4 clip_intersect(const f4& in, const f4& out, float din, float dout)
-{
-    const float t = din / (din - dout);
-    f4 r;
-    r.x = in.x + (out.x - in.x) * t;
-    r.y = in.y + (out.y - in.y) * t;
-    r.z = in.z + (out.z - in.z) * t;
-    r.w = in.w + (out.w - in.w) * t;
-    return r;
-}
-
-#define CLIP_MAXV 10
-#define CLIP_THREADS 64u
-template <uint32_t STRIDE>
-struct ClipLds {
-    float4* poly; float* pu; float* pv; int32_t* px; int32_t* py; float* pd; uint32_t tl;
-    __device__ __forceinline__ float4& P(int bf, int i) const { return poly[((uint32_t)bf * CLIP_MAXV + (uint32_t)i) * STRIDE + tl]; }
-    __device__ __forceinline__ float& U(int bf, int i) const { return pu[((uint32_t)bf * CLIP_MAXV + (uint32_t)i) * STRIDE + tl]; }
-    __device__ __forceinline__ float& V(int bf, int i) const { return pv[((uint32_t)bf * CLIP_MAXV + (uint32_t)i) * STRIDE + tl]; }
-    __device__ __forceinline__ int32_t& X(int i) const { return px[(uint32_t)i * STRIDE + tl]; }
-    __device__ __forceinline__ int32_t& Y(int i) const { return py[(uint32_t)i * STRIDE + tl]; }
-    __device__ __forceinline__ float& D(int i) const { return pd[(uint32_t)i * STRIDE + tl]; }
-};
-
-template <uint32_t STRIDE>
-__device__ __forceinline__ int clip_triangle(const RasterParams& p, const ClipLds<STRIDE>& L, const DMeshlet& m, uint32_t V, uint32_t tri,
-                                             const Mat4& mvp, bool masked, int& cur)
-{
-    const uint32_t packedIdx = p.meshletData[m.dataOffset + V + tri];
-    for (int i = 0; i < 3; i++) {
-        const uint32_t li = (packedIdx >> (8 * i)) & 0xFFu;
-        const uint32_t vi = p.meshletData[m.dataOffset + li] + m.vertexBase;
-        const float* pos = p.positions + (size_t)vi * 3;
-        const f4 h = mul_mv(mvp, pos[0], pos[1], pos[2], 1.0f);
-        L.P(0, i) = make_float4(h.x, h.y, h.z, h.w);
-        float u = 0.0f, v = 0.0f;
-        if (masked && p.texcoords) { u = p.texcoords[(size_t)vi * 2]; v = p.texcoords[(size_t)vi * 2 + 1]; }
-        L.U(0, i) = u; L.V(0, i) = v;
-    }
-    int np = 3;
-    cur = 0;
-    for (int pl = p.depthClamp ? 2 : 0; pl < 6 && np >= 3; pl++) {
-        int m2 = 0;
-        for (int i = 0; i < np; i++) {
-            const int j = (i + 1) % np;
-            const float4 Pv = L.P(cur, i), Qv = L.P(cur, j);
-            const f4 P = {Pv.x, Pv.y, Pv.z, Pv.w}, Q = {Qv.x, Qv.y, Qv.z, Qv.w};
-            const float pui = L.U(cur, i), pvi = L.V(cur, i), puj = L.U(cur, j), pvj = L.V(cur, j);
-            const float dp = clip_dist(P, pl), dq = clip_dist(Q, pl);
-            const bool pin = dp >= 0.0f, qin = dq >= 0.0f;
-            if (pin && m2 < CLIP_MAXV) { L.U(cur ^ 1, m2) = pui; L.V(cur ^ 1, m2) = pvi; L.P(cur ^ 1, m2) = Pv; m2++; }
-            if (pin && !qin && m2 < CLIP_MAXV) {
-                const float t = dp / (dp - dq);
-                L.U(cur ^ 1, m2) = pui + (puj - pui) * t; L.V(cur ^ 1, m2) = pvi + (pvj - pvi) * t;
-                const f4 x = clip_intersect(P, Q, dp, dq);
-                L.P(cur ^ 1, m2) = make_float4(x.x, x.y, x.z, x.w); m2++;
-            } else if (!pin && qin && m2 < CLIP_MAXV) {
-                const float t = dq / (dq - dp);
-                L.U(cur ^ 1, m2) = puj + (pui - puj) * t; L.V(cur ^ 1, m2) = pvj + (pvi - pvj) * t;
-                const f4 x = clip_intersect(Q, P, dq, dp);
-                L.P(cur ^ 1, m2) = make_float4(x.x, x.y, x.z, x.w); m2++;
-            }
-        }
-        np = m2; cur ^= 1;
-    }
-    if (np < 3) return 0;
-    for (int i = 0; i < np; i++) {
-        const float4 h = L.P(cur, i);
-        if (!(h.w > 0.0f)) return 0;
-        const float u = h.x / fabsf(h.w) * 0.5f + 0.5f;
-        const float v = h.y / fabsf(h.w) * -0.5f + 0.5f;
-        L.X(i) = (int32_t)rintf((u * p.W) * 256.0f);
-        L.Y(i) = (int32_t)rintf((v * p.H) * 256.0f);
-        L.D(i) = h.z / h.w;
-    }
-    return np;
 }
 
 __device__ void raster_clip_part(const RasterParams& p, uint32_t block, uint32_t blocks)
@@ -1383,41 +1560,7 @@
     const uint32_t n = min(p.counters->clipTriCount[p.pass], p.clipTriCap);
     const uint32_t listShard = block % CHORD_LIST_SHARDS;
     for (uint32_t k = block * CLIP_THREADS + threadIdx.x; k < n; k += blocks * CLIP_THREADS) {
-        const ClipTri ct = p.clipTris[k];
-        ChordDrawCmd cmd; cmd.objectId = ct.objectId; cmd.meshletId = ct.meshletId; cmd.slot = ct.slot;
-        const DMeshlet& m = p.meshlets[cmd.meshletId];
-        const uint32_t V = m.vertexTriangleCount & 0xFFu;
-        const uint32_t matFlags = p.objStatic[cmd.objectId].matFlags;
-        const bool twoSided = (matFlags & CHORD_MATFLAG_TWO_SIDED) != 0u || p.depthOnly != 0u;
-        const bool masked = CHORD_MATFLAG_ALPHA(matFlags) == CHORD_ALPHA_MASK;
-        const float* mv = p.objFrame[cmd.objectId].mvp;
-        Mat4 mvp;
-        for (int r = 0; r < 4; r++) for (int cc = 0; cc < 4; cc++) mvp.r[r][cc] = mv[r * 4 + cc];
-        int cur;
-        const int np = clip_triangle(p, L, m, V, ct.tri, mvp, masked, cur);
-        if (np < 3) continue;
-        const uint32_t payload = p.depthOnly ? 0u : encode_triangle_instance(ct.tri, cmd.slot);
-        const uint32_t slots = masked ? 1u + CHORD_MASK_EXT_SLOTS : 1u;
-        for (int i = 1; i + 1 < np; i++) {
-            TriSetup ts;
-            ts.X[0] = L.X(0); ts.X[1] = L.X(i); ts.X[2] = L.X(i + 1);
-            ts.Y[0] = L.Y(0); ts.Y[1] = L.Y(i); ts.Y[2] = L.Y(i + 1);
-            float d[3] = {L.D(0), L.D(i), L.D(i + 1)};
-            ts.payload = payload;
-            if (!tri_setup(ts, twoSided, p.Wi, p.Hi) || !owns_rect(p.shard, ts.px0, ts.py0, ts.px1, ts.py1)) continue;
-            if (p.biasConst != 0.0f || p.biasSlope != 0.0f) { const float o = depth_bias(ts, d, p.biasConst, p.biasSlope); d[0] += o; d[1] += o; d[2] += o; }
-            const uint32_t li = atomicAdd(&p.counters->triCount[listShard * CHORD_SHARD_STRIDE], slots);
-            if (li + slots > p.triCap) { atomicOr(&p.counters->overflow, 1u); continue; }
-            const uint32_t gi = listShard * p.triCap + li;
-            write_record(&p.tris[gi], ts, d, twoSided, masked);
-            if (masked) {
-                const uint32_t material = CHORD_MATFLAG_MATERIAL(matFlags);
-                const float u3[3] = {L.U(cur, 0), L.U(cur, i), L.U(cur, i + 1)}, v3[3] = {L.V(cur, 0), L.V(cur, i), L.V(cur, i + 1)};
-                const float w3[3] = {L.P(cur, 0).w, L.P(cur, i).w, L.P(cur, i + 1).w};
-                write_mask_ext(&p.tris[gi + 1u], &p.materials[material], material, ts.area, u3, v3, w3);
-            }
-            bin_record_tiles(p, ts, gi | (masked ? CHORD_REC_MASKED : CHORD_REC_WIDE));
-        }
+        clip_entry<true>(p, L, p.clipTris[k], listShard);
     }
 }
 
@@ -2834,6 +2977,8 @@
     p.tilesX = c->tilesX; p.tilesY = c->tilesY;
     p.clipTris = c->dClipTris + (size_t)pass * (c->clipTriCap / 2); p.clipTriCap = c->clipTriCap / 2; p.pass = pass;
     p.largeList = c->dLargeList + (size_t)pass * (c->largeCap / 2); p.largeCap = c->largeCap / 2 / CHORD_LIST_SHARDS;
+    static const bool binInSetup = [] { const char* e = getenv("CHORDVIS_BIN_IN_SETUP"); return !e || atoi(e) != 0; }();
+    p.binInSetup = binInSetup ? 1u : 0u;
     p.counters = c->dCounters;
     p.clearTiles = clearTiles ? 1u : 0u;
     p.depthOnly = c->depthOnly ? 1u : 0u; p.depthClamp = c->depthClamp ? 1u : 0u;
@@ -2914,7 +3059,7 @@
     if (c->anyMasked) CHORD_LAUNCH(c, raster_setup_kernel<true>, dim3(blocks), dim3(256), 0, c->stream, p);
     else              CHORD_LAUNCH(c, raster_setup_kernel<false>, dim3(blocks), dim3(256), 0, c->stream, p);
     stamp(c, S_R_CLUSTER);
-    CHORD_LAUNCH(c, raster_clip_and_bin_large_kernel, dim3(CLIP_BLOCKS + (uint32_t)c->numCUs * 4u), dim3(256), 0, c->stream, p);
+    if (!p.binInSetup) CHORD_LAUNCH(c, raster_clip_and_bin_large_kernel, dim3(CLIP_BLOCKS + (uint32_t)c->numCUs * 4u), dim3(256), 0, c->stream, p);
     bool makeOrder = p.orderKept != 2u;
     p.orderAll = 0u; p.tileOrderNext = nullptr;
     static const bool keepLaterOn = [] { const char* e = getenv("CHORDVIS_TILE_KEEP_LATER"); return !e || atoi(e) != 0; }();
```

After: 3.383 Gtri/s (median of 6 runs). +3.3%, better.
